# facebookresearch/seamless_communication

Measured on AMD Instinct MI355X. Metric: S2ST utterances/sec (and real-time factor), seamlessM4T_v2_large, 10 s audio, higher is better.
Workload: dtype f32 activations x f16 weights, f32 accumulate

## Files before the change

include/seamless_hip.h:

```cpp
#ifndef SEAMLESS_HIP_H_
#define SEAMLESS_HIP_H_

#include <stddef.h>
#include <stdint.h>

#ifdef __cplusplus
extern "C" {
#endif

#define SC_ABI_VERSION 10
#define SC_MAX_UPSAMPLES 8
#define SC_MAX_RESBLOCK_KERNELS 4
#define SC_MAX_RESBLOCK_DILATIONS 4

typedef enum sc_status {
    SC_OK = 0,
    SC_ERR_INVALID = -1,
    SC_ERR_HIP = -2,
    SC_ERR_CAPACITY = -3,
    SC_ERR_INTERNAL = -4
} sc_status;

typedef enum sc_dtype { SC_F16 = 0, SC_F32 = 1, SC_I32 = 2 } sc_dtype;

typedef struct sc_tensor_desc {
    const char* name;
    int32_t dtype;
    int32_t ndim;
    int64_t shape[4];
    const void* data;
    int32_t on_device;
} sc_tensor_desc;

typedef struct sc_config {
    int32_t abi_version;
    int32_t model_dim, num_heads;
    int32_t num_fbank_channels, fbank_stride;
    int32_t enc_layers, enc_ffn_dim, depthwise_conv_kernel_size, shaw_max_left, shaw_max_right;
    int32_t adaptor_kernel_size, adaptor_stride, adaptor_ffn_dim, adaptor_proj_dim;
    int32_t dec_layers, dec_ffn_dim, text_vocab_size, text_max_seq_len;
    int32_t pad_idx, unk_idx, bos_idx, eos_idx;
    int32_t t2u_enc_layers, t2u_dec_layers, t2u_ffn_dim, t2u_conv_kernel, t2u_conv_inner_dim;
    int32_t unit_vocab_size, unit_pad_idx, unit_eos_idx, unit_max_seq_len;
    int32_t char_vocab_size, char_max_seq_len, var_pred_hidden_dim, var_pred_kernel_size;
    int32_t voc_num_upsamples;
    int32_t voc_upsample_rates[SC_MAX_UPSAMPLES];
    int32_t voc_upsample_kernel_sizes[SC_MAX_UPSAMPLES];
    int32_t voc_upsample_initial_channel;
    int32_t voc_num_resblock_kernels;
    int32_t voc_resblock_kernel_sizes[SC_MAX_RESBLOCK_KERNELS];
    int32_t voc_num_resblock_dilations;
    int32_t voc_resblock_dilation_sizes[SC_MAX_RESBLOCK_KERNELS][SC_MAX_RESBLOCK_DILATIONS];
    int32_t voc_num_embeddings, voc_embedding_dim, voc_lang_embedding_dim, voc_num_langs;
    int32_t voc_spkr_embedding_dim, voc_num_spkrs;
    int32_t has_t2u, has_vocoder;
    int32_t text_enc_layers, text_enc_ffn_dim;
    int32_t mma_layers, mma_ffn_dim, mma_energy_layers, mma_pre_decision_ratio;
    float mma_temperature;
    int32_t enc_variant;
    int32_t voc_dur_pred_hidden_dim, voc_dur_pred_kernel_size;
    int32_t t2u_variant;
} sc_config;

typedef struct sc_gen_opts {
    int32_t beam_size;
    float soft_max_seq_len_a;
    int32_t soft_max_seq_len_b;
    int32_t hard_max_seq_len;
    int32_t min_seq_len;
    float unk_penalty;
    int32_t use_graph;
    float len_penalty;
    int32_t normalize_scores;
    int32_t no_repeat_ngram_size;
    int32_t source_len;
} sc_gen_opts;

typedef struct sc_model sc_model;

const char* sc_last_error(void);
int sc_abi_version(void);

sc_model* sc_load(const sc_tensor_desc* tensors, size_t n_tensors, const sc_config* cfg, int device);
sc_model* sc_fork(sc_model* parent);
void sc_free(sc_model* m);
int sc_synchronize(sc_model* m);
int sc_wait_stream(sc_model* m, void* producer_stream);
int sc_set_nar_tables(sc_model* m, int32_t vocab, const int32_t* h_tok_len, const uint8_t* h_starts_space,
                      const uint8_t* h_is_punct, const int64_t* h_char_offsets, const int32_t* h_char_ids);

int sc_fbank(sc_model* m, const float* d_wav, int32_t n, int64_t wav_stride, const int32_t* h_num_samples,
             int32_t standardize, float* d_out, int32_t t_rows, int32_t* h_out_frames);

// ... 112 lines not shown
```

include/seamless_hip_internal.h:

```cpp
#ifndef SEAMLESS_HIP_INTERNAL_H_
#define SEAMLESS_HIP_INTERNAL_H_

#include "seamless_hip.h"

#ifdef __cplusplus
extern "C" {
#endif

int sc_decoder_step_family(sc_model* m, int rows, int caller);

int sc_op_knob(const char* name, int dflt);

int sc_op_force_general_gemm(int on);
int32_t sc_op_voc_pack_plan(const int32_t* h_need, int32_t n, int64_t budget_rows, int32_t* h_group_first, int32_t cap);
int32_t sc_op_voc_tile_first(const int32_t* h_off, int32_t n, int32_t mul, int32_t tile_rows, int32_t* h_first);
int32_t sc_op_last_vocoder_packed_groups(sc_model* m);
int sc_op_single_plane(int on);
int sc_op_layernorm(const float* d_x, const float* d_gamma, const float* d_beta, float* d_y, int32_t rows, int32_t C,
                    int32_t act);
int sc_op_linear(const float* d_x, const void* d_w_f16, const float* d_bias, const float* d_res, float* d_y,
                 int32_t M, int32_t N, int32_t K, int32_t act, float alpha, int32_t split, int32_t force_gemv);
int sc_op_skinny_linear(const float* d_x, const void* d_w_f16, const float* d_bias, const float* d_res, float* d_y,
                        int32_t M, int32_t N, int32_t K, int32_t act, float alpha);
int sc_op_skinny_res_ln(const float* d_in, const void* d_w_f16, const float* d_bias, float* d_x_inout,
                        const float* d_gamma, const float* d_beta, float* d_h, int32_t M, int32_t N, int32_t K,
                        int32_t splits);
int sc_op_skinny_argmax(const float* d_x, const void* d_w_f16, int32_t M, int32_t N, int32_t K, int32_t step,
                        int32_t min_step_for_eos, int32_t force_eos_step, int32_t pad_idx, int32_t eos_idx,
                        int32_t unk_idx, float unk_penalty, int32_t* d_idx, float* d_lprob);

int sc_op_dstep_res_ln(const float* d_in, const void* d_w_f16, const float* d_bias, float* d_x_inout, const float* d_gamma,
                       const float* d_beta, float* d_h, int32_t M, int32_t N, int32_t K, int32_t splits);
int sc_op_dstep_linear_planes(const float* d_x, const void* d_w_f16, const float* d_bias, float* d_y, int32_t M, int32_t N, int32_t K,
                              int32_t act);
int sc_op_dstep_argmax(const float* d_x, const void* d_w_f16, int32_t M, int32_t N, int32_t K, int32_t step,
                       int32_t min_step_for_eos, int32_t force_eos_step, int32_t pad_idx, int32_t eos_idx, int32_t unk_idx,
                       float unk_penalty, int32_t ntl, int32_t* d_idx, float* d_lprob);
int sc_op_dstep_attention(const float* d_proj, int32_t S, const float* d_bias, float* d_kcache, float* d_vcache, int32_t cap,
                          int32_t pos, const int32_t* d_lens, int32_t cross, int32_t nb, int32_t heads, float* d_out);
int sc_op_dstep3_gemv(int32_t mode, const float* d_x, const void* d_w_f16, const float* d_bias, const float* d_gamma,
                      const float* d_beta, const float* d_res, float* d_y, float* d_h, int32_t M, int32_t N, int32_t K, int32_t act,
                      int32_t rg, int32_t shape);
int sc_op_dstep3_argmax(const float* d_x, const void* d_w_f16, int32_t M, int32_t N, int32_t K, int32_t step,
                        int32_t min_step_for_eos, int32_t force_eos_step, int32_t pad_idx, int32_t eos_idx, int32_t unk_idx,
                        float unk_penalty, int32_t* d_idx, float* d_lprob);
int sc_op_chain_bench(int32_t kind, int32_t rows, int32_t n, int32_t reps, float* us_per_kernel);
int sc_op_conv1d(const float* d_x, const void* d_w_f16_packed, const float* d_bias, const float* d_res, float* d_y,
                 int32_t nb, int32_t t_in, int32_t cin, int32_t cout, int32_t k, int32_t stride, int32_t pad,
                 int32_t dil, const int32_t* d_in_lens, int32_t in_act, int32_t act);
int sc_op_pack_conv_weight(const void* d_w_f16, void* d_dst_f16, int32_t cout, int32_t cin, int32_t k);
int sc_op_conv_transpose1d(const float* d_x, const void* d_v_f16, const void* d_g_f16, const float* d_bias,
                           float* d_y, int32_t nb, int32_t t_in, int32_t cin, int32_t cout, int32_t k,
                           int32_t stride, int32_t pad, int32_t in_act);
int sc_op_linear_presplit(const float* d_x, const void* d_w_f16, const float* d_bias, const float* d_res, float* d_y,
                          void* d_yh_f16, void* d_yl_f16, int32_t M, int32_t N, int32_t K, int32_t act, float alpha);
int sc_op_linear_presplit_argmax(const float* d_x, const void* d_w_f16, const float* d_bias, int32_t* d_idx, int32_t M, int32_t N,
                                 int32_t K);
int sc_op_conv1d_presplit(const float* d_x, const void* d_w_f16_packed, const float* d_bias, const float* d_res, float* d_y,
                          void* d_yh_f16, void* d_yl_f16, int32_t nb, int32_t t, int32_t cin, int32_t cout, int32_t k, int32_t pad,
                          int32_t dil, const unsigned char* d_row_valid, int32_t act);
int sc_op_resblock_pair_ps(const float* d_x, const void* d_w1_packed, const float* d_b1, const void* d_w2_packed, const float* d_b2,
                           float* d_out, int32_t nb, int32_t T, int32_t C, int32_t k, int32_t dil);
int sc_op_resblock_pair(const float* d_x, const void* d_w1_packed, const float* d_b1, const void* d_w2_packed,
                        const float* d_b2, float* d_out, int32_t nb, int32_t T, int32_t C, int32_t k, int32_t dil,
                        float slope, const float* d_avg_a, const float* d_avg_b);
int sc_op_mrf_fused(const float* d_x, const void* const* d_w1_packed, const float* const* d_b1, const void* const* d_w2_packed,
                    const float* const* d_b2, float* d_out, int32_t nb, int32_t T, int32_t C, const int32_t* k, const int32_t* dil,
                    float slope);
int sc_op_attention(const float* d_q, const float* d_k, const float* d_v, float* d_out, int32_t nb, int32_t heads,
                    int32_t sq, int32_t skv, int64_t ldq, int64_t ldk, int64_t ldv, int64_t ldo,
                    const int32_t* d_kv_lens, int32_t causal, const float* d_rel_k, int32_t rel_left,
                    int32_t rel_right);
int sc_op_attention_ex(const float* d_q, const float* d_k, const float* d_v, float* d_out, int32_t nb, int32_t heads,
                       int32_t sq, int32_t skv, int64_t ldq, int64_t ldk, int64_t ldv, int64_t ldo,
                       const int32_t* d_kv_lens, int32_t causal, const float* d_rel_k, int32_t rel_left,
                       int32_t rel_right, const int32_t* d_row_off, const float* d_rp_table, int64_t rp_ld,
                       const float* d_q_bias_u, const float* d_q_bias_v, void* d_out_hi, void* d_out_lo, int64_t ldoh);
int sc_op_glu_dwconv(const float* d_x, const float* d_w, float* d_y, int32_t nb, int32_t T, int32_t C, int32_t k,
                     const int32_t* d_lens);
int sc_op_glu_dwconv_ln(const float* d_x, const float* d_w, const float* d_gamma, const float* d_beta, int32_t act, void* d_yh_f16,
                        void* d_yl_f16, int32_t nb, int32_t T, int32_t C, int32_t k, const int32_t* d_lens, int32_t fused);
int sc_op_layernorm2(const float* d_x, const float* d_ga, const float* d_ba, const float* d_gb, const float* d_bb, float* d_y,
                     void* d_yh_f16, void* d_yl_f16, int32_t rows, int32_t C, int32_t fused);
int sc_op_argmax(const float* d_logits, int32_t rows, int32_t V, int32_t* d_idx, float* d_lprob);

int sc_op_beam_candidates(float* d_logits, int64_t ld, int32_t n_utt, int32_t beams, int32_t V, const float* d_cum, int32_t first_step,
                          int32_t no_eos, int32_t force_eos, int32_t pad_idx, int32_t eos_idx, int32_t unk_idx, float unk_penalty, int32_t K,
                          float* d_cand_val, int32_t* d_cand_idx, const int32_t* d_seqs, int32_t seq_ld, int32_t S, int32_t G,
                          const int32_t* d_rows, const int32_t* d_slots, int32_t chunked);
int sc_op_beam_candidates_banned(float* d_logits, int64_t ld, int32_t n_utt, int32_t beams, int32_t V, const float* d_cum,
                                 int32_t first_step, int32_t no_eos, int32_t force_eos, int32_t pad_idx, int32_t eos_idx, int32_t unk_idx,
                                 float unk_penalty, int32_t K, float* d_cand_val, int32_t* d_cand_idx, const int32_t* d_seqs,
                                 int32_t seq_ld, int32_t S, int32_t G, const int32_t* d_rows, const int32_t* d_slots, int32_t chunked,
                                 const int32_t* d_banned_tokens, const int32_t* d_banned_offsets, int32_t n_banned);
int sc_op_beam_select(const float* d_cand_val, const int32_t* d_cand_idx, const int32_t* d_seqs_cur, int32_t* d_seqs_new, float* d_fin_score,
                      int32_t* d_fin_len, int32_t* d_fin_seq, int32_t* d_fin_count, int32_t* d_done, int32_t* d_remaining, int32_t* d_tok,
                      int32_t* d_src_row, float* d_cum, int32_t* d_anc, int32_t anc_ld, const int32_t* d_slot_utt, const int32_t* d_slots,
                      int32_t n, int32_t beams, int32_t K, int32_t V, int32_t max_len, int32_t step, int32_t eos_idx, int32_t pad_idx,
                      int32_t normalize, float len_penalty);
int sc_op_beam_compact(const int32_t* d_done, int32_t* d_slot_utt, int32_t* d_slots, int32_t* d_rows, int32_t* d_seqs, float* d_cum,
                       int32_t* d_tok, int32_t* d_enc_lens, int32_t* d_anc, int32_t n, int32_t beams, int32_t max_len, int32_t anc_ld,
                       int32_t seq_len, int32_t anc_len);
int sc_op_gather_cache(const float* d_src, float* d_dst, const int32_t* d_src_row, int32_t rows, int32_t len, int32_t cap, int32_t M,
                       int32_t layers, int64_t layer_stride);
int sc_op_row_token_lprob(const float* d_logits, int64_t ld, int32_t rows, int32_t V, int32_t row_stride, int32_t token, float* d_out);

int sc_op_dstep_attention_ex(const float* d_proj, int32_t S, const float* d_bias, float* d_kcache, float* d_vcache, int32_t cap,
                             int32_t cache_rows, int32_t pos, const int32_t* d_lens, int32_t cross, int32_t nb, int32_t heads,
                             const int32_t* d_slot_rp, const int32_t* d_slot_lane, const int32_t* d_anc, const int32_t* d_kv_item,
                             int32_t kv_row_div, const int32_t* d_rows, float* d_out);
int sc_op_engine_step_close(const float* d_x, const void* d_w_f16, int32_t M, int32_t N, int32_t K, int32_t min_step_for_eos, int32_t pad_idx,
                            int32_t eos_idx, int32_t unk_idx, float unk_penalty, int32_t* d_slot_rp, const int32_t* d_rows, int32_t n_states,
                            int32_t cap, int32_t* d_tok, int32_t* d_pos, int32_t* d_finished, int32_t* d_out_len, const int32_t* d_limit,
                            const int32_t* d_prefix_len, float* d_score, int32_t* d_hist);
int sc_op_engine_admit(const int32_t* d_recs, int32_t n, int32_t n_states, int32_t cap, int32_t pad_idx, int32_t* d_tok, int32_t* d_pos,
                       int32_t* d_finished, int32_t* d_out_len, int32_t* d_limit, int32_t* d_prefix_len, int32_t* d_enc_lens, float* d_score,
                       int32_t* d_hist);
int sc_op_engine_set_slots(const int32_t* d_rids, int32_t n_live, int32_t slots, int32_t n_states, int32_t* d_slot_rp, int32_t* d_slot_lane,
                           const int32_t* d_pos, int32_t* d_rows);
int sc_op_engine_retire(const int32_t* h_rid, const int32_t* h_dst_rows, float* const* h_dst, int32_t n, int32_t n_states, int32_t cap, int32_t M,
                        const int32_t* d_out_len, const float* d_score, const int32_t* d_hist, const float* d_hidden, int32_t* d_stage);
int sc_op_dstep3_embed_ex(const int32_t* d_tok, const void* d_embed_f16, float scale, const float* d_pos_table, int32_t pos,
                          const int32_t* d_slot_rp, const int32_t* d_rows, int32_t rows, int32_t C, int32_t n_states, int32_t n_pos, int32_t vocab,
                          float* d_x);
int sc_op_dstep3_reduce_capture_ex(const float* d_partial, int32_t S, const float* d_bias, float* d_x_inout, const float* d_gamma, const float* d_beta,
                                   float* d_h, float* d_hrow, int64_t hrow_bs, int32_t hrow_rows, int32_t pos, const int32_t* d_slot_rp,
                                   const int32_t* d_rows, int32_t rows, int32_t C, int32_t n_states);
int sc_op_step_update(int32_t* d_next_tok, int32_t* d_hist, int32_t hist_ld, int32_t* d_finished, int32_t* d_out_len, const float* d_lprob,
                      float* d_score, int32_t nb, int32_t pos, int32_t pad_idx, int32_t eos_idx, int32_t* d_n_unfinished);
int sc_op_row_swap(float* d_k, float* d_v, float* d_cross, int32_t layers, int32_t pairs, const int32_t* h_src, const int32_t* h_dst, int32_t n_rows,
                   int32_t M, int32_t cap, int32_t s_enc, int32_t filled, int32_t* d_tok, int32_t* d_finished, int32_t* d_out_len,
                   int32_t* d_enc_lens, float* d_lprob, float* d_score, int32_t* d_hist, float* d_hidden);
int sc_op_align_lprob(const float* d_text, const float* d_feat, int32_t n, int32_t s_text, int32_t s_feat, int32_t C,
                      const int32_t* h_text_lens, const int32_t* h_feat_lens, float temperature, float* d_lprob);
int sc_op_mas(const float* d_lprob, int32_t n, int32_t s_text, int32_t s_feat, const int32_t* h_text_lens, const int32_t* h_feat_lens,
              int32_t* h_durations);

#ifdef __cplusplus
}
#endif
#endif
```

seamless_communication_amd/_lib.py:

```python
from __future__ import annotations

import ctypes as C
from pathlib import Path
from typing import Optional

import os

_VARIANT = os.environ.get("SC_LIB_VARIANT", "")
LIB_PATH = Path(__file__).resolve().parent / (f"libseamless_hip.{_VARIANT}.so" if _VARIANT else "libseamless_hip.so")

SC_ABI_VERSION = 10
SC_MAX_UPSAMPLES = 8
SC_MAX_RESBLOCK_KERNELS = 4
SC_MAX_RESBLOCK_DILATIONS = 4
SC_F16, SC_F32, SC_I32 = 0, 1, 2


class SeamlessHipError(RuntimeError):
    pass


class sc_tensor_desc(C.Structure):
    _fields_ = [
        ("name", C.c_char_p),
        ("dtype", C.c_int32),
        ("ndim", C.c_int32),
        ("shape", C.c_int64 * 4),
        ("data", C.c_void_p),
        ("on_device", C.c_int32),
    ]


_i = C.c_int32


class sc_config(C.Structure):
    _fields_ = [
        ("abi_version", _i), ("model_dim", _i), ("num_heads", _i),
        ("num_fbank_channels", _i), ("fbank_stride", _i),
        ("enc_layers", _i), ("enc_ffn_dim", _i), ("depthwise_conv_kernel_size", _i),
        ("shaw_max_left", _i), ("shaw_max_right", _i),
        ("adaptor_kernel_size", _i), ("adaptor_stride", _i), ("adaptor_ffn_dim", _i), ("adaptor_proj_dim", _i),
        ("dec_layers", _i), ("dec_ffn_dim", _i), ("text_vocab_size", _i), ("text_max_seq_len", _i),
        ("pad_idx", _i), ("unk_idx", _i), ("bos_idx", _i), ("eos_idx", _i),
        ("t2u_enc_layers", _i), ("t2u_dec_layers", _i), ("t2u_ffn_dim", _i), ("t2u_conv_kernel", _i),
        ("t2u_conv_inner_dim", _i),
        ("unit_vocab_size", _i), ("unit_pad_idx", _i), ("unit_eos_idx", _i), ("unit_max_seq_len", _i),
        ("char_vocab_size", _i), ("char_max_seq_len", _i), ("var_pred_hidden_dim", _i), ("var_pred_kernel_size", _i),
        ("voc_num_upsamples", _i),
        ("voc_upsample_rates", _i * SC_MAX_UPSAMPLES),
        ("voc_upsample_kernel_sizes", _i * SC_MAX_UPSAMPLES),
        ("voc_upsample_initial_channel", _i),
        ("voc_num_resblock_kernels", _i),
        ("voc_resblock_kernel_sizes", _i * SC_MAX_RESBLOCK_KERNELS),
        ("voc_num_resblock_dilations", _i),
        ("voc_resblock_dilation_sizes", (_i * SC_MAX_RESBLOCK_DILATIONS) * SC_MAX_RESBLOCK_KERNELS),
        ("voc_num_embeddings", _i), ("voc_embedding_dim", _i), ("voc_lang_embedding_dim", _i), ("voc_num_langs", _i),
        ("voc_spkr_embedding_dim", _i), ("voc_num_spkrs", _i),
        ("has_t2u", _i), ("has_vocoder", _i),
        ("text_enc_layers", _i), ("text_enc_ffn_dim", _i),
        ("mma_layers", _i), ("mma_ffn_dim", _i), ("mma_energy_layers", _i), ("mma_pre_decision_ratio", _i),
        ("mma_temperature", C.c_float),
        ("enc_variant", _i),
        ("voc_dur_pred_hidden_dim", _i), ("voc_dur_pred_kernel_size", _i),
        ("t2u_variant", _i),
    ]


class sc_gen_opts(C.Structure):
    _fields_ = [
        ("beam_size", _i), ("soft_max_seq_len_a", C.c_float), ("soft_max_seq_len_b", _i),
        ("hard_max_seq_len", _i), ("min_seq_len", _i), ("unk_penalty", C.c_float), ("use_graph", _i),
        ("len_penalty", C.c_float), ("normalize_scores", _i), ("no_repeat_ngram_size", _i), ("source_len", _i),
    ]


class sc_engine_opts(C.Structure):
    _fields_ = [
        ("slots", _i), ("rows", _i), ("max_len", _i), ("s_enc", _i), ("min_seq_len", _i), ("unk_penalty", C.c_float),
        ("poll", _i), ("low_water", _i), ("max_wait_ms", _i), ("use_graph", _i),
    ]


class sc_engine_stats(C.Structure):
    _fields_ = [
        ("steps", C.c_int64), ("row_steps", C.c_int64), ("useful_row_steps", C.c_int64), ("rows_admitted", C.c_int64),
        ("rows_retired", C.c_int64), ("requests", C.c_int64), ("max_live", C.c_int64), ("busy_us", C.c_double), ("wait_us", C.c_double),
        ("self_kv_bytes", C.c_int64), ("cross_kv_bytes", C.c_int64), ("hidden_bytes", C.c_int64),
    ]


class sc_aligner_config(C.Structure):
    _fields_ = [
        ("abi_version", _i), ("model_dim", _i), ("feat_dim", _i), ("text_layers", _i), ("feat_layers", _i),
# ... 8 lines not shown
    "sc_last_error": (C.c_char_p, []),
    "sc_abi_version": (C.c_int, []),
    "sc_load": (_P, [C.POINTER(sc_tensor_desc), C.c_size_t, C.POINTER(sc_config), C.c_int]),
    "sc_fork": (_P, [_P]),
    "sc_free": (None, [_P]),
    "sc_synchronize": (C.c_int, [_P]),
    "sc_wait_stream": (C.c_int, [_P, _P]),
    "sc_decoder_step_family": (C.c_int, [_P, C.c_int, C.c_int]),
    "sc_set_nar_tables": (C.c_int, [_P, _i, _P, _P, _P, _P, _P]),
    "sc_fbank": (C.c_int, [_P, _P, _i, C.c_int64, _P, _i, _P, _i, _P]),
    "sc_fbank_rate": (C.c_int, [_P, _P, _i, C.c_int64, _P, _i, _i, _P, _i, _P]),
    "sc_fbank_frames": (_i, [C.c_int64, _i]),
    "sc_encoder_out_len": (_i, [_P, _i]),
    "sc_encode_speech": (C.c_int, [_P, _P, _i, _i, _P, _P, _P]),
    "sc_encode_text": (C.c_int, [_P, _P, C.c_int32, C.c_int32, _P, _P]),
    "sc_mma_begin": (C.c_int, [_P, _P, C.c_int32, C.c_int32]),
    "sc_mma_step": (C.c_int, [_P, _P, C.c_int32, _P, C.c_int32, _P, _P, _P]),
    "sc_text_max_len": (_i, [_P, C.POINTER(sc_gen_opts), _i]),
    "sc_generate_text": (C.c_int, [_P, _P, _i, _i, _P, C.POINTER(sc_gen_opts), _P, _i, _P, _P, _P, _P]),
    "sc_generate_text_banned": (C.c_int, [_P, _P, _i, _i, _P, C.POINTER(sc_gen_opts), _P, _i, _P, _P, _P, _P, _P, _P, _i]),
    "sc_generate_text_capture": (C.c_int, [_P, _P, _i, _i, _P, C.POINTER(sc_gen_opts), _P, _i, _P, _P, _P, _P, _P, _P]),
    "sc_decode_text": (C.c_int, [_P, _P, _i, _i, _P, _P, _i, _P]),
    "sc_engine_create": (_P, [_P, C.POINTER(sc_engine_opts)]),
    "sc_engine_free": (None, [_P]),
    "sc_engine_attach": (C.c_int, [_P, _P]),
    "sc_engine_expect": (C.c_int, [_P, _i]),
    "sc_engine_get_stats": (C.c_int, [_P, C.POINTER(sc_engine_stats), _i]),
    "sc_t2u_nar": (C.c_int, [_P, _P, _i, _i, _P, _P, C.c_float, _P, _PI, _PI]),
    "sc_get_units": (C.c_int, [_P, _P]),
    "sc_get_durations": (C.c_int, [_P, _P, _P, _P]),
    "sc_vocoder_hop": (_i, [_P]),
    "sc_vocode": (C.c_int, [_P, _P, _i, _i, _P, _P, _P]),
    "sc_vocode_ragged": (C.c_int, [_P, _P, _i, _i, _P, _P, _P, _P]),
    "sc_vocoder_durations": (C.c_int, [_P, _P, _i, _i, _P]),
    "sc_t2u_ar": (C.c_int, [_P, _P, _i, _i, _P, C.POINTER(sc_gen_opts), _P, _i, _P, _i, _P, _P]),
    "sc_t2u_ar_max_len": (_i, [_P, C.POINTER(sc_gen_opts), _i]),
    "sc_last_padding": (C.c_int, [_P, _P, _P, _P]),
    "sc_s2st": (C.c_int, [_P, _P, _i, _i, _P, C.POINTER(sc_gen_opts), _P, _i, C.c_float, _P, _P, _P, _i, _P, _P, _i, _P, _P, _P]),
    "sc_prof_enable": (C.c_int, [C.c_int]),
    "sc_prof_reset": (C.c_int, []),
    "sc_prof_report": (C.c_int64, [C.c_char_p, C.c_int64]),
    "sc_text_to_char_seqs": (C.c_int32, [C.c_int32, _P, _P, _P, _P, _P, C.c_int32, C.c_int32, C.c_int32, _P, C.c_int32, C.c_int32,
                                         _P, _P, C.c_int32, _P]),
    "sc_ngram_blocked_tokens": (C.c_int32, [_PI, C.c_int32, C.c_int32, _PI, C.c_int32]),
    "sc_banned_blocked_tokens": (C.c_int32, [_PI, C.c_int32, _PI, _PI, C.c_int32, _PI, C.c_int32]),
    "sc_aligner_load": (_P, [C.POINTER(sc_tensor_desc), C.c_size_t, C.POINTER(sc_aligner_config), C.c_int]),
    "sc_aligner_free": (None, [_P]),
    "sc_align": (C.c_int, [_P, _P, _i, _i, _P, _P, _i, _P, _P, _P]),
    "sc_op_align_lprob": (C.c_int, [_P, _P, _i, _i, _i, _i, _P, _P, C.c_float, _P]),
    "sc_op_mas": (C.c_int, [_P, _i, _i, _i, _P, _P, _P]),
    "sc_op_knob": (C.c_int, [C.c_char_p, C.c_int]),
    "sc_op_force_general_gemm": (C.c_int, [C.c_int]),
    "sc_op_voc_pack_plan": (C.c_int32, [_PI, C.c_int32, C.c_int64, _PI, C.c_int32]),
    "sc_op_voc_tile_first": (C.c_int32, [_PI, C.c_int32, C.c_int32, C.c_int32, _PI]),
    "sc_op_last_vocoder_packed_groups": (C.c_int32, [_P]),
    "sc_op_single_plane": (C.c_int, [C.c_int]),
    "sc_op_layernorm": (C.c_int, [_P, _P, _P, _P, _i, _i, _i]),
    "sc_op_linear": (C.c_int, [_P, _P, _P, _P, _P, _i, _i, _i, _i, C.c_float, _i, _i]),
    "sc_op_skinny_linear": (C.c_int, [_P, _P, _P, _P, _P, _i, _i, _i, _i, C.c_float]),
    "sc_op_skinny_res_ln": (C.c_int, [_P, _P, _P, _P, _P, _P, _P, _i, _i, _i, _i]),
    "sc_op_skinny_argmax": (C.c_int, [_P, _P, _i, _i, _i, _i, _i, _i, _i, _i, _i, C.c_float, _P, _P]),
    "sc_op_dstep_res_ln": (C.c_int, [_P, _P, _P, _P, _P, _P, _P, _i, _i, _i, _i]),
    "sc_op_dstep_linear_planes": (C.c_int, [_P, _P, _P, _P, _i, _i, _i, _i]),
    "sc_op_dstep_argmax": (C.c_int, [_P, _P, _i, _i, _i, _i, _i, _i, _i, _i, _i, C.c_float, _i, _P, _P]),
    "sc_op_resblock_pair_ps": (C.c_int, [_P, _P, _P, _P, _P, _P, _i, _i, _i, _i, _i]),
    "sc_op_glu_dwconv_ln": (C.c_int, [_P, _P, _P, _P, _i, _P, _P, _i, _i, _i, _i, _P, _i]),
    "sc_op_layernorm2": (C.c_int, [_P, _P, _P, _P, _P, _P, _P, _P, _i, _i, _i]),
    "sc_op_dstep3_gemv": (C.c_int, [_i, _P, _P, _P, _P, _P, _P, _P, _P, _i, _i, _i, _i, _i, _i]),
    "sc_op_dstep3_argmax": (C.c_int, [_P, _P, _i, _i, _i, _i, _i, _i, _i, _i, _i, C.c_float, _P, _P]),
    "sc_op_chain_bench": (C.c_int, [_i, _i, _i, _i, _P]),
    "sc_op_dstep_attention": (C.c_int, [_P, _i, _P, _P, _P, _i, _i, _P, _i, _i, _i, _P]),
    "sc_op_conv1d": (C.c_int, [_P, _P, _P, _P, _P, _i, _i, _i, _i, _i, _i, _i, _i, _P, _i, _i]),
    "sc_op_pack_conv_weight": (C.c_int, [_P, _P, _i, _i, _i]),
    "sc_op_conv_transpose1d": (C.c_int, [_P, _P, _P, _P, _P, _i, _i, _i, _i, _i, _i, _i, _i]),
    "sc_op_linear_presplit": (C.c_int, [_P, _P, _P, _P, _P, _P, _P, _i, _i, _i, _i, C.c_float]),
    "sc_op_linear_presplit_argmax": (C.c_int, [_P, _P, _P, _P, _i, _i, _i]),
    "sc_op_conv1d_presplit": (C.c_int, [_P, _P, _P, _P, _P, _P, _P, _i, _i, _i, _i, _i, _i, _i, _P, _i]),
    "sc_op_mrf_fused": (C.c_int, [_P, _P, _P, _P, _P, _P, _i, _i, _i, _P, _P, C.c_float]),
    "sc_op_resblock_pair": (C.c_int, [_P, _P, _P, _P, _P, _P, _i, _i, _i, _i, _i, C.c_float, _P, _P]),
    "sc_op_attention": (C.c_int, [_P, _P, _P, _P, _i, _i, _i, _i, C.c_int64, C.c_int64, C.c_int64, C.c_int64, _P, _i,
                                  _P, _i, _i]),
    "sc_op_attention_ex": (C.c_int, [_P, _P, _P, _P, _i, _i, _i, _i, C.c_int64, C.c_int64, C.c_int64, C.c_int64, _P, _i,
                                     _P, _i, _i, _P, _P, C.c_int64, _P, _P, _P, _P, C.c_int64]),
    "sc_op_glu_dwconv": (C.c_int, [_P, _P, _P, _i, _i, _i, _i, _P]),
    "sc_op_argmax": (C.c_int, [_P, _i, _i, _P, _P]),
    "sc_op_beam_candidates": (C.c_int, [_P, C.c_int64, _i, _i, _i, _P, _i, _i, _i, _i, _i, _i, C.c_float, _i, _P, _P, _P, _i, _i, _i,
                                        _P, _P, _i]),
    "sc_op_beam_candidates_banned": (C.c_int, [_P, C.c_int64, _i, _i, _i, _P, _i, _i, _i, _i, _i, _i, C.c_float, _i, _P, _P, _P, _i, _i,
                                               _i, _P, _P, _i, _P, _P, _i]),
    "sc_op_beam_select": (C.c_int, [_P, _P, _P, _P, _P, _P, _P, _P, _P, _P, _P, _P, _P, _P, _i, _P, _P, _i, _i, _i, _i, _i, _i, _i, _i,
                                    _i, C.c_float]),
    "sc_op_beam_compact": (C.c_int, [_P, _P, _P, _P, _P, _P, _P, _P, _P, _i, _i, _i, _i, _i, _i]),
    "sc_op_gather_cache": (C.c_int, [_P, _P, _P, _i, _i, _i, _i, _i, C.c_int64]),
    "sc_op_row_token_lprob": (C.c_int, [_P, C.c_int64, _i, _i, _i, _i, _P]),
    "sc_op_dstep_attention_ex": (C.c_int, [_P, _i, _P, _P, _P, _i, _i, _i, _P, _i, _i, _i, _P, _P, _P, _P, _i, _P, _P]),
    "sc_op_engine_step_close": (C.c_int, [_P, _P, _i, _i, _i, _i, _i, _i, _i, C.c_float, _P, _P, _i, _i, _P, _P, _P, _P, _P, _P, _P, _P]),
    "sc_op_engine_admit": (C.c_int, [_P, _i, _i, _i, _i, _P, _P, _P, _P, _P, _P, _P, _P, _P]),
    "sc_op_engine_set_slots": (C.c_int, [_P, _i, _i, _i, _P, _P, _P, _P]),
    "sc_op_engine_retire": (C.c_int, [_P, _P, _P, _i, _i, _i, _i, _P, _P, _P, _P, _P]),
    "sc_op_dstep3_embed_ex": (C.c_int, [_P, _P, C.c_float, _P, _i, _P, _P, _i, _i, _i, _i, _i, _P]),
    "sc_op_dstep3_reduce_capture_ex": (C.c_int, [_P, _i, _P, _P, _P, _P, _P, _P, C.c_int64, _i, _i, _P, _P, _i, _i, _i]),
    "sc_op_step_update": (C.c_int, [_P, _P, _i, _P, _P, _P, _P, _i, _i, _i, _i, _P]),
    "sc_op_row_swap": (C.c_int, [_P, _P, _P, _i, _i, _P, _P, _i, _i, _i, _i, _i, _P, _P, _P, _P, _P, _P, _P, _P]),
}

_lib: Optional[C.CDLL] = None


def load_library() -> C.CDLL:
    global _lib
    if _lib is not None:
        return _lib
    if not LIB_PATH.exists():
        raise SeamlessHipError(
            f"{LIB_PATH} is missing: build it with `python -m seamless_communication_amd.build` "
            "(there is no CPU fallback for the HIP path)"
        )
    lib = C.CDLL(str(LIB_PATH))
    for name, (res, args) in SIGNATURES.items():
        fn = getattr(lib, name)
        fn.restype = res
        fn.argtypes = args
    if lib.sc_abi_version() != SC_ABI_VERSION:
        raise SeamlessHipError(f"ABI mismatch: library {lib.sc_abi_version()} vs binding {SC_ABI_VERSION}")
    _lib = lib
    return lib


def banned_csr(banned_seqs):
    import numpy as np

    seqs = [[int(t) for t in (s.tolist() if hasattr(s, "tolist") else s)] for s in banned_seqs]
    if any(len(s) == 0 for s in seqs):
        raise ValueError("a banned sequence must hold at least one token")
    off = np.zeros(len(seqs) + 1, dtype=np.int32)
    off[1:] = np.cumsum([len(s) for s in seqs], dtype=np.int64)
    tok = np.asarray([t for s in seqs for t in s], dtype=np.int32)
    return tok, off


def check(status: int, what: str) -> None:
    if status != 0:
        msg = load_library().sc_last_error()
        raise SeamlessHipError(f"{what} failed with status {status}: {msg.decode() if msg else '?'}")


def make_config(cfg, has_t2u: bool = True, has_vocoder: bool = True, has_text_encoder: bool = False,
                has_monotonic_decoder: bool = False, has_vocoder_dur_predictor: bool = False) -> sc_config:
    c = sc_config()
    c.abi_version = SC_ABI_VERSION
    for f in (
        "model_dim num_heads num_fbank_channels fbank_stride enc_layers enc_ffn_dim depthwise_conv_kernel_size "
        "shaw_max_left shaw_max_right adaptor_kernel_size adaptor_stride adaptor_ffn_dim adaptor_proj_dim dec_layers "
        "dec_ffn_dim text_vocab_size text_max_seq_len pad_idx unk_idx bos_idx eos_idx t2u_enc_layers t2u_dec_layers "
        "t2u_ffn_dim t2u_conv_kernel t2u_conv_inner_dim unit_vocab_size unit_pad_idx unit_eos_idx unit_max_seq_len "
        "char_vocab_size char_max_seq_len var_pred_hidden_dim var_pred_kernel_size"
    ).split():
        setattr(c, f, int(getattr(cfg, f)))
    v = cfg.vocoder
    if len(v.upsample_rates) > SC_MAX_UPSAMPLES or len(v.resblock_kernel_sizes) > SC_MAX_RESBLOCK_KERNELS:
        raise ValueError("vocoder config exceeds the ABI's fixed array sizes")
    c.voc_num_upsamples = len(v.upsample_rates)
    for i, (r, k) in enumerate(zip(v.upsample_rates, v.upsample_kernel_sizes)):
        c.voc_upsample_rates[i] = r
        c.voc_upsample_kernel_sizes[i] = k
    c.voc_upsample_initial_channel = v.upsample_initial_channel
# ... 30 lines not shown
```

seamless_communication_amd/csrc/api.hip:

```cpp
#include <atomic>
#include <cstring>
#include <map>
#include <mutex>
#include <set>

#include "../../include/seamless_hip_internal.h"
#include "engine.h"
#include "model.h"

using namespace sc;

struct sc_model {
    Model m;
};

struct sc_engine {
    std::unique_ptr<Engine> e;
    int device = 0;
    const void* weights = nullptr;
    std::set<sc_model*> attached;
};

static std::mutex g_attach_mu;
static std::map<Engine*, sc_engine*> g_engine_owner;
// ... 1030 lines not shown
        if (kind == 7) one(i & 1 ? 1 : 2);
        else one(kind);
    }
    SC_HIP(hipStreamEndCapture(st, &g));
    SC_HIP(hipGraphInstantiate(&ge, g, nullptr, nullptr, 0));
    for (int r = 0; r < 2; ++r) SC_HIP(hipGraphLaunch(ge, st));
    SC_HIP(hipStreamSynchronize(st));
    hipEvent_t e0, e1;
    SC_HIP(hipEventCreate(&e0));
    SC_HIP(hipEventCreate(&e1));
    SC_HIP(hipEventRecord(e0, st));
    for (int r = 0; r < reps; ++r) SC_HIP(hipGraphLaunch(ge, st));
    SC_HIP(hipEventRecord(e1, st));
    SC_HIP(hipStreamSynchronize(st));
    float ms = 0.f;
    SC_HIP(hipEventElapsedTime(&ms, e0, e1));
    *us_per_kernel = 1e3f * ms / (float)(reps * n);
    (void)hipEventDestroy(e0);
    (void)hipEventDestroy(e1);
    (void)hipGraphExecDestroy(ge);
    (void)hipGraphDestroy(g);
    (void)hipStreamDestroy(st);
    SC_API_END
}

int sc_op_pack_conv_weight(const void* d_w_f16, void* d_dst_f16, int32_t cout, int32_t cin, int32_t k) {
    SC_API_BEGIN
    const int kpad = (int)align_up((int64_t)cin * k, 32);
    launch_pack_conv_weight(static_cast<const __half*>(d_w_f16), static_cast<__half*>(d_dst_f16), cout, cin, k, kpad,
                            g_op_stream);
    SC_HIP(hipStreamSynchronize(g_op_stream));
    SC_API_END
}

int sc_op_conv1d(const float* d_x, const void* d_w_f16_packed, const float* d_bias, const float* d_res, float* d_y,
                 int32_t nb, int32_t t_in, int32_t cin, int32_t cout, int32_t k, int32_t stride, int32_t pad, int32_t dil,
                 const int32_t* d_in_lens, int32_t in_act, int32_t act) {
    SC_API_BEGIN
    Model tmp;
    Conv c;
    c.w = static_cast<const __half*>(d_w_f16_packed);
    c.b = d_bias;
    c.cout = cout;
    c.cin = cin;
    c.k = k;
    c.kpad = (int)align_up((int64_t)cin * k, 32);
    conv1d(tmp, d_x, c, d_res, d_y, nb, t_in, stride, pad, dil, d_in_lens, in_act, act);
    SC_HIP(hipStreamSynchronize(g_op_stream));
    SC_API_END
}

int sc_op_conv_transpose1d(const float* d_x, const void* d_v_f16, const void* d_g_f16, const float* d_bias, float* d_y,
                           int32_t nb, int32_t t_in, int32_t cin, int32_t cout, int32_t k, int32_t stride, int32_t pad,
                           int32_t in_act) {
    SC_API_BEGIN
    SC_CHECK(pad == (k - stride) / 2 && k - 2 * pad == stride, "sc_op_conv_transpose1d: unsupported geometry");
    Model tmp;
    ConvT c;
    c.cin = cin;
    c.cout = cout;
    c.k = k;
    c.stride = stride;
    c.pad = pad;
    c.taps = cdiv(k, stride);
    c.kpad = (int)align_up((int64_t)cin * c.taps, 32);
    float* folded = nullptr;
    __half* packed = nullptr;
    SC_HIP(hipMalloc(&folded, (size_t)cin * cout * k * 4));
    SC_HIP(hipMalloc(&packed, (size_t)stride * cout * c.kpad * 2));
    launch_weight_norm_fold(static_cast<const __half*>(d_v_f16), static_cast<const __half*>(d_g_f16), folded, cin, cout * k,
                            g_op_stream);
    launch_pack_convT_weight(folded, packed, cin, cout, k, stride, c.kpad, g_op_stream);
    c.w = packed;
    c.b = d_bias;
    conv_transpose1d(tmp, d_x, c, d_y, nb, t_in, in_act);
    SC_HIP(hipStreamSynchronize(g_op_stream));
    (void)hipFree(folded);
    (void)hipFree(packed);
    SC_API_END
}

int sc_op_linear_presplit(const float* d_x, const void* d_w_f16, const float* d_bias, const float* d_res, float* d_y,
                          void* d_yh_f16, void* d_yl_f16, int32_t M, int32_t N, int32_t K, int32_t act, float alpha) {
    SC_API_BEGIN
    SC_CHECK(d_x && d_w_f16 && (d_y || d_yh_f16), "sc_op_linear_presplit: null argument");
    __half *hi = nullptr, *lo = nullptr;
    SC_HIP(hipMalloc(&hi, (size_t)M * K * 2));
    SC_HIP(hipMalloc(&lo, (size_t)M * K * 2));
    try {
        launch_split_f32(d_x, hi, lo, (int64_t)M * K, g_op_stream);
        GemmPsArgs a;
        a.Ah = hi;
        a.Al = lo;
        a.lda = K;
        a.W = static_cast<const __half*>(d_w_f16);
        a.ldw = K;
        a.bias = d_bias;
        a.res = d_res;
        a.ldr = N;
        a.C = d_y;
        a.ldc = N;
        a.Ch = static_cast<__half*>(d_yh_f16);
        a.Cl = static_cast<__half*>(d_yl_f16);
        a.ldcs = N;
        a.M = M;
        a.N = N;
        a.K = K;
        a.act = act;
        a.alpha = alpha;
        launch_gemm_presplit(a, g_op_stream);
        SC_HIP(hipStreamSynchronize(g_op_stream));
    } catch (...) {
        (void)hipFree(hi);
        (void)hipFree(lo);
        throw;
    }
    (void)hipFree(hi);
    (void)hipFree(lo);
    SC_API_END
}

int sc_op_linear_presplit_argmax(const float* d_x, const void* d_w_f16, const float* d_bias, int32_t* d_idx, int32_t M, int32_t N,
                                 int32_t K) {
    SC_API_BEGIN
    SC_CHECK(d_x && d_w_f16 && d_idx, "sc_op_linear_presplit_argmax: null argument");
    __half *hi = nullptr, *lo = nullptr;
    float2* part = nullptr;
    const int nch = gemm_presplit_amax_chunks(M, N);
    SC_HIP(hipMalloc(&hi, (size_t)M * K * 2));
    SC_HIP(hipMalloc(&lo, (size_t)M * K * 2));
    SC_HIP(hipMalloc(&part, (size_t)M * nch * sizeof(float2)));
    try {
        SC_HIP(hipMemsetAsync(part, 0xff, (size_t)M * nch * sizeof(float2), g_op_stream));
        launch_split_f32(d_x, hi, lo, (int64_t)M * K, g_op_stream);
        GemmPsArgs a;
        a.Ah = hi;
        a.Al = lo;
        a.lda = K;
        a.W = static_cast<const __half*>(d_w_f16);
        a.ldw = K;
        a.bias = d_bias;
        a.M = M;
        a.N = N;
        a.K = K;
        a.amax = part;
        a.amax_ld = nch;
        launch_gemm_presplit(a, g_op_stream);
        launch_amax_finish(part, nch, M, d_idx, g_op_stream);
        SC_HIP(hipStreamSynchronize(g_op_stream));
    } catch (...) {
        (void)hipFree(hi);
        (void)hipFree(lo);
        (void)hipFree(part);
        throw;
    }
    (void)hipFree(hi);
    (void)hipFree(lo);
    (void)hipFree(part);
    SC_API_END
}

int sc_op_conv1d_presplit(const float* d_x, const void* d_w_f16_packed, const float* d_bias, const float* d_res, float* d_y,
                          void* d_yh_f16, void* d_yl_f16, int32_t nb, int32_t t, int32_t cin, int32_t cout, int32_t k, int32_t pad,
                          int32_t dil, const unsigned char* d_row_valid, int32_t act) {
    SC_API_BEGIN
    SC_CHECK(d_x && d_w_f16_packed && (d_y || d_yh_f16), "sc_op_conv1d_presplit: null argument");
    __half *hi = nullptr, *lo = nullptr;
    const size_t n = (size_t)nb * t * cin;
    SC_HIP(hipMalloc(&hi, n * 2));
    SC_HIP(hipMalloc(&lo, n * 2));
    try {
        launch_split_f32(d_x, hi, lo, (int64_t)n, g_op_stream);
        Model tmp;
        Conv c;
        c.w = static_cast<const __half*>(d_w_f16_packed);
        c.b = d_bias;
        c.cout = cout;
        c.cin = cin;
        c.k = k;
        c.kpad = (int)align_up((int64_t)cin * k, 32);
        conv1d_presplit(tmp, hi, lo, c, d_res, d_y, static_cast<__half*>(d_yh_f16), static_cast<__half*>(d_yl_f16), nb, t, pad, dil,
                        d_row_valid, act);
        SC_HIP(hipStreamSynchronize(g_op_stream));
    } catch (...) {
        (void)hipFree(hi);
        (void)hipFree(lo);
        throw;
// ... 55 lines not shown
int sc_op_mrf_fused(const float* d_x, const void* const* d_w1_packed, const float* const* d_b1, const void* const* d_w2_packed,
                    const float* const* d_b2, float* d_out, int32_t nb, int32_t T, int32_t C, const int32_t* k, const int32_t* dil,
                    float slope) {
    SC_API_BEGIN
    SC_CHECK(d_x && d_w1_packed && d_b1 && d_w2_packed && d_b2 && d_out && k && dil, "sc_op_mrf_fused: null argument");
    MrfArgs a;
    a.x = d_x;
    a.out = d_out;
    a.nb = nb;
    a.T = T;
    a.C = C;
    a.slope = slope;
    for (int j = 0; j < 3; ++j) a.k[j] = k[j];
    for (int q = 0; q < 9; ++q) {
        a.dil[q] = dil[q];
        a.w1[q] = static_cast<const __half*>(d_w1_packed[q]);
        a.w2[q] = static_cast<const __half*>(d_w2_packed[q]);
        a.ldw1[q] = a.ldw2[q] = align_up((int64_t)C * k[q / 3], 32);
        a.b1[q] = d_b1[q];
        a.b2[q] = d_b2[q];
    }
    a.single = g_op_single.load();
    launch_mrf_fused(a, g_op_stream);
    SC_HIP(hipStreamSynchronize(g_op_stream));
    SC_API_END
}

int sc_op_attention(const float* d_q, const float* d_k, const float* d_v, float* d_out, int32_t nb, int32_t heads,
                    int32_t sq, int32_t skv, int64_t ldq, int64_t ldk, int64_t ldv, int64_t ldo, const int32_t* d_kv_lens,
                    int32_t causal, const float* d_rel_k, int32_t rel_left, int32_t rel_right) {
    SC_API_BEGIN
    AttnArgs a;
    a.q = d_q;
    a.k = d_k;
    a.v = d_v;
    a.out = d_out;
    a.ldq = ldq;
    a.ldk = ldk;
    a.ldv = ldv;
    a.ldo = ldo;
    a.nb = nb;
    a.heads = heads;
    a.Sq = sq;
    a.Skv = skv;
    a.kv_lens = d_kv_lens;
    a.causal = causal;
    a.rel_k = d_rel_k;
    a.rel_left = rel_left;
    a.rel_right = rel_right;
    launch_attention(a, g_op_stream);
    SC_HIP(hipStreamSynchronize(g_op_stream));
    SC_API_END
}

int sc_op_attention_ex(const float* d_q, const float* d_k, const float* d_v, float* d_out, int32_t nb, int32_t heads,
                       int32_t sq, int32_t skv, int64_t ldq, int64_t ldk, int64_t ldv, int64_t ldo, const int32_t* d_kv_lens,
                       int32_t causal, const float* d_rel_k, int32_t rel_left, int32_t rel_right, const int32_t* d_row_off,
                       const float* d_rp_table, int64_t rp_ld, const float* d_q_bias_u, const float* d_q_bias_v, void* d_out_hi,
                       void* d_out_lo, int64_t ldoh) {
    SC_API_BEGIN
    AttnArgs a;
    a.q = d_q;
    a.k = d_k;
    a.v = d_v;
    a.out = d_out;
    a.ldq = ldq;
    a.ldk = ldk;
    a.ldv = ldv;
    a.ldo = ldo;
    a.nb = nb;
    a.heads = heads;
    a.Sq = sq;
    a.Skv = skv;
    a.kv_lens = d_kv_lens;
    a.causal = causal;
    a.rel_k = d_rel_k;
    a.rel_left = rel_left;
    a.rel_right = rel_right;
    a.row_off = d_row_off;
    a.rp_table = d_rp_table;
    a.rp_ld = rp_ld;
    a.q_bias_u = d_q_bias_u;
    a.q_bias_v = d_q_bias_v;
    a.out_hi = static_cast<__half*>(d_out_hi);
    a.out_lo = static_cast<__half*>(d_out_lo);
    a.ldoh = ldoh;
    launch_attention(a, g_op_stream);
    SC_HIP(hipStreamSynchronize(g_op_stream));
    SC_API_END
}

int sc_op_glu_dwconv(const float* d_x, const float* d_w, float* d_y, int32_t nb, int32_t T, int32_t C, int32_t k,
                     const int32_t* d_lens) {
    SC_API_BEGIN
    launch_glu_dwconv(d_x, 2 * C, d_w, d_y, C, nb, T, C, k, d_lens, g_op_stream);
    SC_HIP(hipStreamSynchronize(g_op_stream));
    SC_API_END
}

int sc_op_glu_dwconv_ln(const float* d_x, const float* d_w, const float* d_gamma, const float* d_beta, int32_t act, void* d_yh_f16,
                        void* d_yl_f16, int32_t nb, int32_t T, int32_t C, int32_t k, const int32_t* d_lens, int32_t fused) {
    SC_API_BEGIN
    SC_CHECK(d_x && d_w && d_gamma && d_beta && d_yh_f16 && d_yl_f16, "sc_op_glu_dwconv_ln: null argument");
    __half* yh = static_cast<__half*>(d_yh_f16);
    __half* yl = static_cast<__half*>(d_yl_f16);
    if (fused) {
        launch_glu_dwconv_ln(d_x, 2 * C, d_w, d_gamma, d_beta, act, yh, yl, C, nb, T, C, k, d_lens, g_op_stream);
    } else {
        OpScratch scratch;
        float* mid = scratch.get<float>((size_t)nb * T * C);
        launch_glu_dwconv(d_x, 2 * C, d_w, mid, C, nb, T, C, k, d_lens, g_op_stream);
        launch_layernorm_split(mid, C, d_gamma, d_beta, yh, yl, C, nb * T, C, act, nullptr, 1, g_op_stream);
        SC_HIP(hipStreamSynchronize(g_op_stream));
    }
    SC_HIP(hipStreamSynchronize(g_op_stream));
    SC_API_END
}

int sc_op_layernorm2(const float* d_x, const float* d_ga, const float* d_ba, const float* d_gb, const float* d_bb, float* d_y,
                     void* d_yh_f16, void* d_yl_f16, int32_t rows, int32_t C, int32_t fused) {
    SC_API_BEGIN
    SC_CHECK(d_x && d_ga && d_ba && d_gb && d_bb && d_y && d_yh_f16 && d_yl_f16, "sc_op_layernorm2: null argument");
    __half* yh = static_cast<__half*>(d_yh_f16);
    __half* yl = static_cast<__half*>(d_yl_f16);
    if (fused) {
        launch_layernorm2_split(d_x, C, d_ga, d_ba, d_y, C, d_gb, d_bb, yh, yl, C, rows, C, g_op_stream);
    } else {
        launch_layernorm(d_x, C, d_ga, d_ba, d_y, C, rows, C, ACT_NONE, nullptr, 1, g_op_stream);
        launch_layernorm_split(d_y, C, d_gb, d_bb, yh, yl, C, rows, C, ACT_NONE, nullptr, 1, g_op_stream);
    }
    SC_HIP(hipStreamSynchronize(g_op_stream));
    SC_API_END
}

int sc_op_argmax(const float* d_logits, int32_t rows, int32_t V, int32_t* d_idx, float* d_lprob) {
    SC_API_BEGIN
    launch_argmax_rows(d_logits, V, rows, V, nullptr, -1, -1, -1, -1, -1, 0.f, d_idx, d_lprob, g_op_stream);
    SC_HIP(hipStreamSynchronize(g_op_stream));
    SC_API_END
}


static int op_beam_candidates(float* d_logits, int64_t ld, int32_t n_utt, int32_t beams, int32_t V, const float* d_cum, int32_t first_step,
                              int32_t no_eos, int32_t force_eos, int32_t pad_idx, int32_t eos_idx, int32_t unk_idx, float unk_penalty, int32_t K,
                              float* d_cand_val, int32_t* d_cand_idx, const int32_t* d_seqs, int32_t seq_ld, int32_t S, int32_t G,
                              const int32_t* d_rows, const int32_t* d_slots, int32_t chunked, const int32_t* d_banned_tokens,
                              const int32_t* d_banned_offsets, int32_t n_banned) {
    SC_API_BEGIN
    BannedList bl;
    if (n_banned != 0) {
        SC_CHECK(n_banned > 0 && n_banned <= BANNED_MAX_SEQS && d_banned_tokens && d_banned_offsets && d_seqs,
                 "sc_op_beam_candidates_banned: bad banned list (n_banned=%d; needs d_seqs)", n_banned);
        const std::vector<int32_t> off = op_read_ints(d_banned_offsets, (size_t)n_banned + 1);
        SC_CHECK(off[0] == 0 && off[n_banned] >= 0 && off[n_banned] <= BANNED_MAX_TOKENS, "sc_op_beam_candidates_banned: bad offsets");
        for (int q = 0; q < n_banned; ++q) SC_CHECK(off[q + 1] >= off[q], "sc_op_beam_candidates_banned: offsets decrease at %d", q);
        const std::vector<int32_t> tok = op_read_ints(d_banned_tokens, (size_t)off[n_banned]);
        validate_banned_host(tok.data(), off.data(), n_banned, V, &bl.max_len);
        bl.tokens = d_banned_tokens, bl.offsets = d_banned_offsets, bl.n = n_banned;
    }
    const BannedList* banned = bl.n > 0 ? &bl : nullptr;
    SC_CHECK(d_logits && d_cum && d_cand_val && d_cand_idx && n_utt >= 1 && V >= 1 && ld >= V, "sc_op_beam_candidates: bad arguments");
    SC_CHECK(!d_seqs || (G >= 0 && S >= 0 && seq_ld >= S), "sc_op_beam_candidates: bad n-gram arguments (S=%d G=%d seq_ld=%d)", S, G, seq_ld);
    if (d_slots) SC_CHECK(op_read_ints(d_slots, 1)[0] <= n_utt, "sc_op_beam_candidates: *d_slots > n_utt");
    if (chunked) {
        SC_CHECK(beam_chunked(V, beams, K), "sc_op_beam_candidates: the chunked search does not take V=%d beams=%d K=%d", V, beams, K);
        if (d_rows) SC_CHECK(op_read_ints(d_rows, 1)[0] <= n_utt * beams, "sc_op_beam_candidates: *d_rows > n_utt * beams");
// ... 384 lines not shown
```

seamless_communication_amd/csrc/common.cpp:

```cpp
#include "common.h"
#include <cstdlib>
#include <cstring>

namespace sc {

static thread_local char g_err[1024] = "";

void set_error(const char* fmt, ...) {
    va_list ap;
    va_start(ap, fmt);
    vsnprintf(g_err, sizeof(g_err), fmt, ap);
    va_end(ap);
}

const char* get_error() { return g_err; }

namespace knob {
namespace {
struct Knob {
    const char* name;
    int kind;
    const char* what;
};
const Knob knob_table[] = {
    {"SC_DEBUG_NUMERICS", 0, "honour the switches that change results"},
    {"SC_DEBUG_FILL", 0, "fill fresh scratch blocks with NaN (tests)"},
    {"SC_SPLIT_MODE", 1, "1: Conformer products on the hi fp16 plane only (precision study)"},
    {"SC_DECODER_GEN1", 1, "decoder step on the first-generation kernels"},
    {"SC_DECODER_GEN2", 1, "decoder step on the second-generation chain"},
    {"SC_DECODE_STEPWISE", 1, "teacher-forced pass step by step instead of one batched forward"},
    {"SC_VOC_SPLIT", 1, "vocoder ResBlock products on both fp16 planes of their activations again (bit 0 wide stages, bit 2 narrow stages); default: hi plane only"},
    {"SC_GEMM_GENERAL", 0, "general GEMM kernel instead of the fast path"}, {"SC_GEMM_PF2", 0, "GEMM prefetch depth"},
    {"SC_GEMM_GROUP_M", 0, "GEMM workgroup order"}, {"SC_GEMM_TILE", 0, "GEMM tile override"},
    {"SC_PS_TILE", 0, "DMA GEMM: largest tile"}, {"SC_PS_MIN256", 0, "DMA GEMM: tiles needed for 256 x 256"},
    {"SC_PS_MIN128", 0, "DMA GEMM: tiles needed for 128 x 128"},
    {"SC_PRESPLIT", 0, "0: Conformer operands split on the fly"}, {"SC_ENC_FUSE", 0, "0: separate Conformer element-wise launches"},
    {"SC_D3_RG_SMALL", 0, "decoder step: rows per row group, N = 1024 products"}, {"SC_D3_RG_FFN", 0, "decoder step: rows per row group, FFN-in"},
    {"SC_G3_STATIONARY", 0, "row-group products of wide steps: 0 one workgroup per row group, n = workgroup budget of the weight-stationary launch"},
    {"SC_G3_TILES", 0, "0: FFN-out of wide steps on the weight-stationary row-group walk instead of tile-owning waves"},
    {"SC_G3_TOUCH", 0, "weight-stationary products: bit 0 cooperative L2 touch of the activations, bit 1 K slices per XCD (FFN-out); default 3"},
    {"SC_D3_FFN_IN", 0, "decoder step: FFN-in workgroup shape"}, {"SC_D3_FFN_OUT", 0, "decoder step: FFN-out workgroup shape"},
    {"SC_T2U_GROUPS", 0, "NAR T2U: length buckets"}, {"SC_T2U_PACKED", 0, "0: NAR decoder on padded buckets"},
    {"SC_VOC_PS", 0, "0: vocoder wide stages on the register-staged convolution"}, {"SC_VOC_MRF", 0, "0: narrow vocoder stages as nine pair launches"},
    {"SC_VOC_GROUPS", 0, "vocoder: length buckets"}, {"SC_VOC_GROUP_OVERHEAD", 0, "vocoder: bucket planning overhead rows"},
    {"SC_VOC_STREAMS", 0, "vocoder: side chains"},
    {"SC_VOC_PACKED", 0, "0: ragged vocoder batches in length buckets on side chains instead of the packed pass"},
    {"SC_VOC_PACK_ROWS", 0, "vocoder: unit rows per packed group"},
    {"SC_ENGINE_RG_SMALL", 0, "decode engine: rows per row group, N = 1024 products"},
    {"SC_BEAM_COMPACT", 2, "0: beam search keeps finished utterances' slots"},
    {"SC_GREEDY_COMPACT", 2, "0: greedy generation keeps finished rows in their slots"}, {"SC_GREEDY_POLL", 2, "steps between looks at the finished flags"},
};
constexpr int N_KNOBS = sizeof(knob_table) / sizeof(knob_table[0]);
struct State {
    bool set[N_KNOBS];
    int val[N_KNOBS];
    bool numerics = false;
};
const State& state() {
    static const State st = [] {
        State s{};
        const char* dn = getenv("SC_DEBUG_NUMERICS");
        s.numerics = dn && atoi(dn) != 0;
        for (int i = 0; i < N_KNOBS; ++i) {
            const char* e = getenv(knob_table[i].name);
            s.set[i] = e != nullptr && (knob_table[i].kind != 1 || s.numerics);
            s.val[i] = e ? atoi(e) : 0;
        }
        return s;
    }();
    return st;
}
int lookup(const char* name) {
    for (int i = 0; i < N_KNOBS; ++i)
        if (strcmp(knob_table[i].name, name) == 0) return i;
    return -1;
}
int find(const char* name) {
    const int i = lookup(name);
    if (i >= 0) return i;
    fprintf(stderr, "libseamless_hip: switch %s is not in the knob table (common.cpp)\n", name);
    abort();
}
}

bool known(const char* name) { return name && lookup(name) >= 0; }

int value(const char* name, int dflt) {
    const int i = find(name);
    return state().set[i] ? state().val[i] : dflt;
}
bool is_set(const char* name) { return state().set[find(name)]; }
int live(const char* name, int dflt) {
    (void)find(name);
    const char* e = getenv(name);
    return e ? atoi(e) : dflt;
}
void report_once() {
    static const bool done = [] {
        const State& s = state();
        for (int i = 0; i < N_KNOBS; ++i) {
            const char* e = getenv(knob_table[i].name);
            if (!e || knob_table[i].kind == 2) continue;
            if (knob_table[i].kind == 1 && !s.numerics)
                fprintf(stderr, "libseamless_hip: %s=%s IGNORED - it changes results (%s); set SC_DEBUG_NUMERICS=1 to honour it\n", knob_table[i].name, e,
                        knob_table[i].what);
            else
                fprintf(stderr, "libseamless_hip: %s=%s (%s)%s\n", knob_table[i].name, e, knob_table[i].what, knob_table[i].kind == 1 ? " - RESULTS CHANGE" : "");
        }
        return true;
    }();
    (void)done;
}
}

}
```

seamless_communication_amd/csrc/k_attn.hip:

```cpp
#include <cstdlib>

#include "kernels.h"

namespace sc {

static constexpr int HD = 64;

static constexpr int MQ = 128;
static constexpr int MKV = 32;
static constexpr int KS = 68;
typedef _Float16 a16_h8 __attribute__((ext_vector_type(8)));
typedef _Float16 a16_h4 __attribute__((ext_vector_type(4)));
static constexpr int KH_LD = 72;
static constexpr int VT_LD = 40;

__device__ __forceinline__ void a16_split8(const float* x, a16_h8& hi, a16_h8& lo) {
#pragma unroll
    for (int e = 0; e < 8; ++e) {
        const _Float16 h = (_Float16)x[e];
        hi[e] = h;
        lo[e] = (_Float16)(x[e] - (float)h);
    }
}

template <int MODE>
__global__ __launch_bounds__(256) void attn_mfma16_kernel(AttnArgs p) {
    constexpr bool SHAW = MODE == 1;
    constexpr bool RELPOS = MODE == 2;
    typedef float f16v __attribute__((ext_vector_type(16)));
    typedef float f4v __attribute__((ext_vector_type(4)));
    extern __shared__ __attribute__((aligned(16))) float smem[];
    _Float16* sKh = reinterpret_cast<_Float16*>(smem);
    _Float16* sKl = sKh + MKV * KH_LD;
    _Float16* sVh = sKl + MKV * KH_LD;
    _Float16* sVl = sVh + HD * VT_LD;
    float* sQR = smem + 4 * 32 * KS;
    float* sT = smem + 4 * 32 * KS;
    float* sR = smem;

    const int tid = threadIdx.x, lane = tid & 63, wave = tid >> 6;
    const int ql = lane & 31, hh = lane >> 5;
    int qb = blockIdx.x, h = blockIdx.y, n = blockIdx.z;
    {
        const int gx = gridDim.x, bh_all = gridDim.y * gridDim.z;
        if ((bh_all & 7) == 0) {
            const int L = blockIdx.x + gx * (blockIdx.y + gridDim.y * blockIdx.z);
            const int bh = (L / (8 * gx)) * 8 + (L & 7);
            qb = (L >> 3) % gx;
            h = bh % gridDim.y;
            n = bh / gridDim.y;
        }
    }
    const int q0 = qb * MQ + wave * 32;
    const int qi = q0 + ql;
    const int kv_len = p.kv_lens ? min(p.kv_lens[n], p.Skv) : p.Skv;
    const int shift = p.Skv - p.Sq;
    const int qabs = qi + shift;
    const int npos = p.rel_left + 1 + p.rel_right;
    const int sq_n = p.row_off ? kv_len : p.Sq;
    const int64_t qbase = p.row_off ? (int64_t)p.row_off[n] : (int64_t)n * p.Sq;
    const int64_t kvbase = p.row_off ? (int64_t)p.row_off[n] : (int64_t)n * p.Skv;
    if (p.row_off && qb * MQ >= kv_len) return;
    const bool qok = qi < sq_n;
    const float* qrow = p.q + (qbase + (qok ? qi : 0)) * p.ldq + h * HD;

    if (SHAW) {
        float qreg[32];
#pragma unroll
        for (int g = 0; g < 8; ++g) {
            f4v v = {0.f, 0.f, 0.f, 0.f};
            if (qok) v = *reinterpret_cast<const f4v*>(qrow + 8 * g + 4 * hh);
            qreg[4 * g + 0] = v[0];
            qreg[4 * g + 1] = v[1];
            qreg[4 * g + 2] = v[2];
            qreg[4 * g + 3] = v[3];
        }
        for (int idx = tid; idx < npos * (HD / 4); idx += 256) {
            const int r = idx >> 4, c4 = idx & 15;
            *reinterpret_cast<f4v*>(&sR[r * KS + c4 * 4]) = *reinterpret_cast<const f4v*>(p.rel_k + r * HD + c4 * 4);
        }
        __syncthreads();
#pragma unroll 1
        for (int f = 0; f < 3; ++f) {
            if (f * 32 >= npos) break;
            f16v qr;
#pragma unroll
            for (int r = 0; r < 16; ++r) qr[r] = 0.f;
#pragma unroll
            for (int g = 0; g < 8; ++g) {
                const f4v r4 = *reinterpret_cast<const f4v*>(&sR[(f * 32 + ql) * KS + 8 * g + 4 * hh]);
                qr = __builtin_amdgcn_mfma_f32_32x32x2f32(r4[0], qreg[4 * g + 0], qr, 0, 0, 0);
                qr = __builtin_amdgcn_mfma_f32_32x32x2f32(r4[1], qreg[4 * g + 1], qr, 0, 0, 0);
                qr = __builtin_amdgcn_mfma_f32_32x32x2f32(r4[2], qreg[4 * g + 2], qr, 0, 0, 0);
                qr = __builtin_amdgcn_mfma_f32_32x32x2f32(r4[3], qreg[4 * g + 3], qr, 0, 0, 0);
            }
#pragma unroll
            for (int r = 0; r < 16; ++r) {
                const int e = f * 32 + (r & 3) + 8 * (r >> 2) + 4 * hh;
                if (e < npos) sQR[(wave * 32 + ql) * npos + e] = qr[r];
            }
        }
    }

    a16_h8 qh[4], qlo[4], qvh[RELPOS ? 4 : 1], qvl[RELPOS ? 4 : 1];
#pragma unroll
    for (int c = 0; c < 4; ++c) {
        float x[8];
#pragma unroll
        for (int e = 0; e < 8; ++e) x[e] = 0.f;
        if (qok) {
            const f4v v0 = *reinterpret_cast<const f4v*>(qrow + 16 * c + 8 * hh);
            const f4v v1 = *reinterpret_cast<const f4v*>(qrow + 16 * c + 8 * hh + 4);
#pragma unroll
            for (int e = 0; e < 4; ++e) {
                x[e] = v0[e];
                x[4 + e] = v1[e];
            }
        }
        if (RELPOS) {
            float xu[8], xv[8];
#pragma unroll
            for (int e = 0; e < 8; ++e) {
                xu[e] = x[e] + p.q_bias_u[h * HD + 16 * c + 8 * hh + e];
                xv[e] = x[e] + p.q_bias_v[h * HD + 16 * c + 8 * hh + e];
            }
            a16_split8(xu, qh[c], qlo[c]);
            a16_split8(xv, qvh[c], qvl[c]);
        } else {
            a16_split8(x, qh[c], qlo[c]);
        }
    }

    f16v o0, o1;
#pragma unroll
    for (int r = 0; r < 16; ++r) {
        o0[r] = 0.f;
        o1[r] = 0.f;
    }
    float m_i = -1e30f, l_i = 0.f;

    int k_end = kv_len;
    if (p.causal) k_end = min(k_end, qb * MQ + MQ - 1 + shift + 1);

    const int sr0 = tid >> 4, sc4 = tid & 15;
    f4v kf[2], vf[2];
    auto fetch = [&](int k0) {
#pragma unroll
        for (int u = 0; u < 2; ++u) {
            const int r = sr0 + 16 * u;
            kf[u] = f4v{0.f, 0.f, 0.f, 0.f};
            vf[u] = kf[u];
            if (k0 + r < kv_len) {
                const int64_t row = kvbase + k0 + r;
                kf[u] = *reinterpret_cast<const f4v*>(p.k + row * p.ldk + h * HD + sc4 * 4);
                vf[u] = *reinterpret_cast<const f4v*>(p.v + row * p.ldv + h * HD + sc4 * 4);
            }
        }
    };
    if (k_end > 0) fetch(0);

    for (int k0 = 0; k0 < k_end; k0 += MKV) {
        __syncthreads();
#pragma unroll
        for (int u = 0; u < 2; ++u) {
            const int r = sr0 + 16 * u;
            a16_h4 khi, klo, vhi, vlo;
#pragma unroll
            for (int e = 0; e < 4; ++e) {
                const _Float16 a = (_Float16)kf[u][e];
                khi[e] = a;
                klo[e] = (_Float16)(kf[u][e] - (float)a);
                const _Float16 b = (_Float16)vf[u][e];
                vhi[e] = b;
                vlo[e] = (_Float16)(vf[u][e] - (float)b);
            }
            *reinterpret_cast<a16_h4*>(&sKh[r * KH_LD + 4 * sc4]) = khi;
            *reinterpret_cast<a16_h4*>(&sKl[r * KH_LD + 4 * sc4]) = klo;
            const int w = r & 15;
            const int pos = (r & 16) + 8 * ((w >> 2) & 1) + (w & 3) + 4 * (w >> 3);
#pragma unroll
            for (int e = 0; e < 4; ++e) {
                sVh[(4 * sc4 + e) * VT_LD + pos] = vhi[e];
                sVl[(4 * sc4 + e) * VT_LD + pos] = vlo[e];
            }
        }
        if (k0 + MKV < k_end) fetch(k0 + MKV);
        __syncthreads();

        float qr[16];
        if (SHAW) {
            const float* qrow_t = sQR + (wave * 32 + ql) * npos;
            const int rel_max = k0 + (MKV - 1) - (q0 + shift);
            const int rel_min = k0 - (q0 + 31 + shift);
            if (rel_max <= -p.rel_left) {
                const float v = qrow_t[0];
#pragma unroll
                for (int r = 0; r < 16; ++r) qr[r] = v;
            } else if (rel_min >= p.rel_right) {
                const float v = qrow_t[npos - 1];
#pragma unroll
                for (int r = 0; r < 16; ++r) qr[r] = v;
            } else {
#pragma unroll
                for (int r = 0; r < 16; ++r) {
                    const int kj = k0 + (r & 3) + 8 * (r >> 2) + 4 * hh;
                    const int rel = max(-p.rel_left, min(p.rel_right, kj - qabs)) + p.rel_left;
                    qr[r] = qrow_t[rel];
                }
            }
        }
        if (RELPOS) {
            const int t0w = (p.Skv - 1) - (q0 + shift) + k0 - 31;
            const int t_max = 2 * p.Skv - 2;
            float* tw = sT + wave * (64 * 32);
#pragma unroll
            for (int blk = 0; blk < 2; ++blk) {
                const int trow = min(max(t0w + blk * 32 + ql, 0), t_max);
                const float* rrow = p.rp_table + (int64_t)trow * p.rp_ld + h * HD + 8 * hh;
                f4v ra[4][2];
#pragma unroll
                for (int c = 0; c < 4; ++c) {
                    ra[c][0] = *reinterpret_cast<const f4v*>(rrow + 16 * c);
                    ra[c][1] = *reinterpret_cast<const f4v*>(rrow + 16 * c + 4);
                }
                f16v tt;
#pragma unroll
                for (int r = 0; r < 16; ++r) tt[r] = 0.f;
#pragma unroll
                for (int c = 0; c < 4; ++c) {
                    float x[8];
#pragma unroll
                    for (int e = 0; e < 4; ++e) {
                        x[e] = ra[c][0][e];
                        x[4 + e] = ra[c][1][e];
                    }
                    a16_h8 rh, rl;
                    a16_split8(x, rh, rl);
                    tt = __builtin_amdgcn_mfma_f32_32x32x16_f16(rh, qvh[c], tt, 0, 0, 0);
                    tt = __builtin_amdgcn_mfma_f32_32x32x16_f16(rh, qvl[c], tt, 0, 0, 0);
                    tt = __builtin_amdgcn_mfma_f32_32x32x16_f16(rl, qvh[c], tt, 0, 0, 0);
                }
#pragma unroll
                for (int r = 0; r < 16; ++r) tw[(blk * 32 + (r & 3) + 8 * (r >> 2) + 4 * hh) * 32 + ql] = tt[r];
            }
#pragma unroll
            for (int r = 0; r < 16; ++r) {
                const int jl = (r & 3) + 8 * (r >> 2) + 4 * hh;
                qr[r] = tw[(jl - ql + 31) * 32 + ql];
            }
        }
        f16v st;
#pragma unroll
        for (int r = 0; r < 16; ++r) st[r] = 0.f;
#pragma unroll
        for (int c = 0; c < 4; ++c) {
            const a16_h8 kh = *reinterpret_cast<const a16_h8*>(&sKh[ql * KH_LD + 16 * c + 8 * hh]);
            const a16_h8 kl = *reinterpret_cast<const a16_h8*>(&sKl[ql * KH_LD + 16 * c + 8 * hh]);
            st = __builtin_amdgcn_mfma_f32_32x32x16_f16(kh, qh[c], st, 0, 0, 0);
            st = __builtin_amdgcn_mfma_f32_32x32x16_f16(kh, qlo[c], st, 0, 0, 0);
            st = __builtin_amdgcn_mfma_f32_32x32x16_f16(kl, qh[c], st, 0, 0, 0);
        }
        float mx = -INFINITY;
#pragma unroll
        for (int r = 0; r < 16; ++r) {
            const int kj = k0 + (r & 3) + 8 * (r >> 2) + 4 * hh;
            float sc = st[r];
            if (SHAW || RELPOS) sc += qr[r];
            const bool ok = (kj < kv_len) && (!p.causal || kj <= qabs);
            sc = sc * 0.125f + (ok ? 0.f : -INFINITY);
            st[r] = sc;
            mx = fmaxf(mx, sc);
        }
        mx = fmaxf(mx, __shfl_xor(mx, 32));
        const float m_new = fmaxf(m_i, mx);
        constexpr float LOG2E = 1.44269504088896340736f;
        const float alpha = __builtin_amdgcn_exp2f((m_i - m_new) * LOG2E);
        float rs = 0.f;
#pragma unroll
        for (int r = 0; r < 16; ++r) {
            const float pv = __builtin_amdgcn_exp2f((st[r] - m_new) * LOG2E);
            st[r] = pv;
            rs += pv;
        }
        rs += __shfl_xor(rs, 32);
        l_i = l_i * alpha + rs;
        m_i = m_new;
        if (__builtin_amdgcn_ballot_w64(alpha != 1.f) != 0) {
#pragma unroll
            for (int r = 0; r < 16; ++r) {
                o0[r] *= alpha;
                o1[r] *= alpha;
            }
        }
#pragma unroll
        for (int c = 0; c < 2; ++c) {
            float x[8];
#pragma unroll
            for (int e = 0; e < 8; ++e) x[e] = st[8 * c + e];
            a16_h8 ph, pl;
            a16_split8(x, ph, pl);
            const a16_h8 v0h = *reinterpret_cast<const a16_h8*>(&sVh[ql * VT_LD + 16 * c + 8 * hh]);
            const a16_h8 v0l = *reinterpret_cast<const a16_h8*>(&sVl[ql * VT_LD + 16 * c + 8 * hh]);
            const a16_h8 v1h = *reinterpret_cast<const a16_h8*>(&sVh[(32 + ql) * VT_LD + 16 * c + 8 * hh]);
            const a16_h8 v1l = *reinterpret_cast<const a16_h8*>(&sVl[(32 + ql) * VT_LD + 16 * c + 8 * hh]);
            o0 = __builtin_amdgcn_mfma_f32_32x32x16_f16(v0h, ph, o0, 0, 0, 0);
            o1 = __builtin_amdgcn_mfma_f32_32x32x16_f16(v1h, ph, o1, 0, 0, 0);
            o0 = __builtin_amdgcn_mfma_f32_32x32x16_f16(v0h, pl, o0, 0, 0, 0);
            o1 = __builtin_amdgcn_mfma_f32_32x32x16_f16(v1h, pl, o1, 0, 0, 0);
            o0 = __builtin_amdgcn_mfma_f32_32x32x16_f16(v0l, ph, o0, 0, 0, 0);
            o1 = __builtin_amdgcn_mfma_f32_32x32x16_f16(v1l, ph, o1, 0, 0, 0);
        }
    }

    __syncthreads();
    float* ot = smem + wave * (32 * KS);
    const float inv = l_i > 0.f ? 1.0f / l_i : 0.f;
#pragma unroll
    for (int r = 0; r < 16; ++r) {
        const int d = (r & 3) + 8 * (r >> 2) + 4 * hh;
        ot[ql * KS + d] = o0[r] * inv;
        ot[ql * KS + 32 + d] = o1[r] * inv;
    }
#pragma unroll
    for (int it = 0; it < 8; ++it) {
        const int row = it * 4 + (lane >> 4);
        const int c0 = (lane & 15) * 4;
        const int qq = q0 + row;
        const f4v of = *reinterpret_cast<const f4v*>(&ot[row * KS + c0]);
        if (qq >= sq_n) continue;
        if (p.out_hi) {
            const a16_h4 hi = __builtin_convertvector(of, a16_h4);
            const f4v back = __builtin_convertvector(hi, f4v);
            const int64_t off = (qbase + qq) * p.ldoh + h * HD + c0;
            *reinterpret_cast<a16_h4*>(p.out_hi + off) = hi;
            *reinterpret_cast<a16_h4*>(p.out_lo + off) = __builtin_convertvector(of - back, a16_h4);
        } else {
            *reinterpret_cast<f4v*>(p.out + (qbase + qq) * p.ldo + h * HD + c0) = of;
        }
    }
}

static bool g_attn_attr_set = false;

void launch_attention(const AttnArgs& a, hipStream_t s) {
    SC_CHECK(a.nb > 0 && a.heads > 0 && a.Sq > 0 && a.Skv > 0, "attention: empty problem");
    SC_CHECK(a.out || (a.out_hi && a.out_lo && a.ldoh % 4 == 0), "attention: no output");
    SC_CHECK(a.ldq % 4 == 0 && a.ldk % 4 == 0 && a.ldv % 4 == 0 && a.ldo % 4 == 0 && (reinterpret_cast<uintptr_t>(a.out) & 15) == 0,
             "attention: row strides must be multiples of 4 and the output 16-byte aligned");
    const int npos = a.rel_left + 1 + a.rel_right;
    SC_CHECK(npos <= 96, "attention: %d relative positions > 96", npos);
    SC_CHECK(!a.row_off || (a.kv_lens && a.Sq == a.Skv && !a.causal), "attention: packed rows need kv_lens and Sq == Skv");
    if (a.rp_table)
        SC_CHECK(!a.rel_k && !a.causal && a.Sq == a.Skv && a.q_bias_u && a.q_bias_v && a.rp_ld % 4 == 0,
                 "attention: relative positions need self-attention (Sq == Skv), both query biases and a 16-byte aligned table");
    if (!g_attn_attr_set) {
        SC_HIP(hipFuncSetAttribute(reinterpret_cast<const void*>(&attn_mfma16_kernel<0>), hipFuncAttributeMaxDynamicSharedMemorySize, 120 * 1024));
        SC_HIP(hipFuncSetAttribute(reinterpret_cast<const void*>(&attn_mfma16_kernel<1>), hipFuncAttributeMaxDynamicSharedMemorySize, 120 * 1024));
        SC_HIP(hipFuncSetAttribute(reinterpret_cast<const void*>(&attn_mfma16_kernel<2>), hipFuncAttributeMaxDynamicSharedMemorySize, 120 * 1024));
        g_attn_attr_set = true;
    }
    const double pairs = a.pairs > 0 ? a.pairs : (double)a.nb * a.Sq * a.Skv;
    prof::Scope scope(a.rel_k ? "attention_shaw" : "attention", 4.0 * a.heads * pairs * HD,
                      4.0 * a.nb * a.heads * HD * (2.0 * a.Sq + 2.0 * a.Skv), s);
    size_t lds = (size_t)(4 * 32 * KS) * sizeof(float);
    if (a.rel_k) lds += (size_t)(MQ * npos) * sizeof(float);
    if (a.rp_table) lds += (size_t)(4 * 64 * 32) * sizeof(float);
    dim3 grid(cdiv(a.Sq, MQ), a.heads, a.nb);
    if (a.rp_table) hipLaunchKernelGGL((attn_mfma16_kernel<2>), grid, dim3(256), lds, s, a);
    else if (a.rel_k) hipLaunchKernelGGL((attn_mfma16_kernel<1>), grid, dim3(256), lds, s, a);
    else hipLaunchKernelGGL((attn_mfma16_kernel<0>), grid, dim3(256), lds, s, a);
    SC_LAUNCH_CHECK();
}

static constexpr int MAX_CACHE = 4096;

__global__ __launch_bounds__(256) void decode_attn_kernel(
    const float* __restrict__ q, int64_t ldq, const float* __restrict__ k_new,
    const float* __restrict__ v_new, int64_t ldkv, float* __restrict__ kcache,
    float* __restrict__ vcache, int64_t cache_ld, int64_t cache_bs, int cap, float* __restrict__ out,
    int64_t ldo, int heads, const int* __restrict__ d_pos, const int* __restrict__ kv_lens, int use_lens,
    int in_splits, int64_t in_split_stride, const float* __restrict__ bias_q,
    const float* __restrict__ bias_k, const float* __restrict__ bias_v) {
    __shared__ float s_q[HD];
    __shared__ float s_sc[MAX_CACHE];
    __shared__ float s_red[8];
    __shared__ float s_part[4][HD];

    const int tid = threadIdx.x, lane = tid & 63, wave = tid >> 6;
    const int h = blockIdx.x, b = blockIdx.y;
    const int pos = d_pos ? *d_pos : 0;
    const int kv_len = use_lens ? min(kv_lens[b], cap) : pos + 1;
    float* kc = kcache + (int64_t)b * cache_bs + h * HD;
    float* vc = vcache + (int64_t)b * cache_bs + h * HD;
    if (tid < 3 * HD) {
        const int which = tid >> 6, d = tid & 63;
        if (which == 0 || k_new) {
            const float* src = which == 0 ? q : (which == 1 ? k_new : v_new);
            const int64_t ld = which == 0 ? ldq : ldkv;
            const float* bias = which == 0 ? bias_q : (which == 1 ? bias_k : bias_v);
            float v = 0.f;
            for (int sp = 0; sp < in_splits; ++sp) v += src[(int64_t)sp * in_split_stride + (int64_t)b * ld + h * HD + d];
            if (bias) v += bias[h * HD + d];
            if (which == 0) s_q[d] = v;
            else if (which == 1) kc[(int64_t)pos * cache_ld + d] = v;
            else vc[(int64_t)pos * cache_ld + d] = v;
        }
    }
    __syncthreads();
    const int sub = lane & 15, grp = lane >> 4;
    const float4 q4 = *reinterpret_cast<const float4*>(&s_q[sub * 4]);
    float lmax = -INFINITY;
    for (int j0 = 0; j0 < kv_len; j0 += 16) {
        const int j = j0 + wave * 4 + grp;
        float d = 0.f;
        if (j < kv_len) {
            const float4 kv = *reinterpret_cast<const float4*>(kc + (int64_t)j * cache_ld + sub * 4);
            d = fmaf(q4.x, kv.x, d);
            d = fmaf(q4.y, kv.y, d);
            d = fmaf(q4.z, kv.z, d);
            d = fmaf(q4.w, kv.w, d);
        }
#pragma unroll
        for (int off = 8; off > 0; off >>= 1) d += __shfl_xor(d, off);
        if (j < kv_len) {
            d *= 0.125f;
            if (sub == 0) s_sc[j] = d;
            lmax = fmaxf(lmax, d);
        }
    }
#pragma unroll
    for (int off = 32; off > 0; off >>= 1) lmax = fmaxf(lmax, __shfl_xor(lmax, off));
    if (lane == 0) s_red[wave] = lmax;
    __syncthreads();
    const float mx = fmaxf(fmaxf(s_red[0], s_red[1]), fmaxf(s_red[2], s_red[3]));
    float lsum = 0.f;
    for (int j = tid; j < kv_len; j += 256) {
        const float e = expf(s_sc[j] - mx);
        s_sc[j] = e;
        lsum += e;
    }
#pragma unroll
    for (int off = 32; off > 0; off >>= 1) lsum += __shfl_xor(lsum, off);
    if (lane == 0) s_red[4 + wave] = lsum;
    __syncthreads();
    const float denom = (s_red[4] + s_red[5]) + (s_red[6] + s_red[7]);
    float acc = 0.f;
    for (int j = wave; j < kv_len; j += 4) acc = fmaf(s_sc[j], vc[(int64_t)j * cache_ld + lane], acc);
    s_part[wave][lane] = acc;
    __syncthreads();
    if (tid < HD) {
        const float v = (s_part[0][tid] + s_part[1][tid]) + (s_part[2][tid] + s_part[3][tid]);
// ... 20 lines not shown
```

seamless_communication_amd/csrc/k_gemm_ps.hip:

```cpp
#include <cstdlib>
#include <type_traits>

#include "kernels.h"

namespace sc {

typedef _Float16 half8_t __attribute__((ext_vector_type(8)));
typedef float float16_t __attribute__((ext_vector_type(16)));

namespace {

constexpr int PBK = 32;
#define SC_LDS_PTR(p) ((__attribute__((address_space(3))) void*)(p))

template <int ACT>
__device__ __forceinline__ float ps_act(float v) {
    if (ACT == ACT_RELU) return v > 0.f ? v : 0.f;
    if (ACT == ACT_SILU) return v / (1.f + expf(-v));
    if (ACT == ACT_TANH) return tanhf(v);
    return v;
}

typedef int i32x4_t __attribute__((ext_vector_type(4)));

__device__ __forceinline__ i32x4_t make_rsrc_words(const void* base, uint32_t bytes) {
    const uint64_t b = reinterpret_cast<uint64_t>(base);
    i32x4_t r;
    r[0] = __builtin_amdgcn_readfirstlane((int)(uint32_t)b);
    r[1] = __builtin_amdgcn_readfirstlane((int)(uint32_t)((b >> 32) & 0xffff));
    r[2] = __builtin_amdgcn_readfirstlane((int)bytes);
    r[3] = 0x00020000;
    return r;
}

__device__ __forceinline__ int swz(int row, int s) { return row * 64 + ((s ^ ((row >> 2) & 3)) << 4); }

template <int WM, int WN, int EP_LD, int ACT>
__device__ __forceinline__ void ps_epilogue(const GemmPsArgs& p, const float* ep, int m0w, int n0w, int lane) {
    typedef float f4_t __attribute__((ext_vector_type(4)));
    typedef _Float16 h4_t __attribute__((ext_vector_type(4)));
    constexpr int LPR = WN / 4;
    constexpr int RPG = 16 / LPR;
    constexpr int RPI = 4 * RPG;
    const int l5 = lane & 31;
    const bool g1 = (l5 >= 4 && l5 < 12) || (l5 >= 16 && l5 < 20) || l5 >= 28;
    const int rank = g1 ? (l5 < 12 ? l5 - 4 : l5 < 20 ? l5 - 8 : l5 - 16) : (l5 < 4 ? l5 : l5 < 16 ? l5 - 8 : l5 - 12);
    const int grp = (lane >> 5) * 2 + (g1 ? 1 : 0);
    const int row_in = grp * RPG + rank / LPR;
    const int c0 = (rank % LPR) * 4;
    const int col = n0w + c0;
    const bool vec_ok = (col + 3 < p.N) && ((p.ldc | p.ldr | p.ldcs) % 4 == 0) && (n0w % 4 == 0);
    f4_t b4 = {0.f, 0.f, 0.f, 0.f};
    if (p.bias) {
#pragma unroll
        for (int e = 0; e < 4; ++e) b4[e] = (col + e < p.N) ? p.bias[col + e] : 0.f;
    }
#pragma unroll
    for (int it = 0; it < WM / RPI; ++it) {
        const int row = it * RPI + row_in;
        const int64_t m = m0w + row;
        const f4_t a = *reinterpret_cast<const f4_t*>(ep + row * EP_LD + c0);
        if (m >= p.M || col >= p.N) continue;
        const bool dead = p.row_valid && p.row_valid[m] == 0;
        f4_t v;
#pragma unroll
        for (int e = 0; e < 4; ++e) v[e] = dead ? 0.f : ps_act<ACT>(a[e] + b4[e]) * p.alpha;
        if (vec_ok) {
            if (p.res && !dead) v += *reinterpret_cast<const f4_t*>(p.res + m * p.ldr + col);
            if (p.C) *reinterpret_cast<f4_t*>(p.C + m * p.ldc + col) = v;
            if (p.Ch) {
                if (p.plane_neg_slope != 1.0f) {
#pragma unroll
                    for (int e = 0; e < 4; ++e) v[e] = fmaxf(v[e], 0.f) + p.plane_neg_slope * fminf(v[e], 0.f);
                }
                const h4_t hi = __builtin_convertvector(v, h4_t);
                *reinterpret_cast<h4_t*>(reinterpret_cast<_Float16*>(p.Ch) + m * p.ldcs + col) = hi;
                if (p.Cl)
                    *reinterpret_cast<h4_t*>(reinterpret_cast<_Float16*>(p.Cl) + m * p.ldcs + col) =
                        __builtin_convertvector(v - __builtin_convertvector(hi, f4_t), h4_t);
            }
        } else {
#pragma unroll
            for (int e = 0; e < 4; ++e) {
                if (col + e >= p.N) continue;
                float x = v[e];
                if (p.res && !dead) x += p.res[m * p.ldr + col + e];
                if (p.C) p.C[m * p.ldc + col + e] = x;
                if (p.Ch) {
                    if (p.plane_neg_slope != 1.0f) x = fmaxf(x, 0.f) + p.plane_neg_slope * fminf(x, 0.f);
                    const _Float16 h = (_Float16)x;
                    reinterpret_cast<_Float16*>(p.Ch)[m * p.ldcs + col + e] = h;
                    if (p.Cl) reinterpret_cast<_Float16*>(p.Cl)[m * p.ldcs + col + e] = (_Float16)(x - (float)h);
                }
            }
        }
    }
}

template <int BM, int BN, int WGM, int WGN, bool SPLIT, bool CONV, bool AMAX>
__global__ __launch_bounds__(WGM* WGN * 64) void gemm_ps_kernel(GemmPsArgs p, int tiles_n, int tiles_total, int tiles_per_xcd,
                                                                 uint32_t a_bytes, uint32_t w_bytes) {
    constexpr int NWAVE = WGM * WGN;
    constexpr bool ALTERNATE = SPLIT && NWAVE == 8;
    constexpr bool MID_BARRIER = SPLIT && !ALTERNATE;
    constexpr int WM = BM / WGM, WN = BN / WGN;
    constexpr int TM = WM / 32, TN = WN / 32;
    constexpr int ACH = BM / (16 * NWAVE);
    constexpr int BCH = BN / (16 * NWAVE);
    constexpr uint32_t OOB = 0x80000000u;
    constexpr int A_TILE = BM * 32, B_TILE = BN * 32;

    constexpr int A_PL = SPLIT ? 2 : 1;
    constexpr int STAGE_BYTES = (A_PL * A_TILE + B_TILE) * 2;
    constexpr int EPN = WN < 64 ? WN : (NWAVE * WM * (64 + 4) * 4 <= 3 * STAGE_BYTES ? 64 : 32);
    constexpr int EP_LD = EPN + 4;
    static_assert(NWAVE * WM * EP_LD * 4 <= 3 * STAGE_BYTES, "epilogue tiles must fit in the stage memory");
    __shared__ __attribute__((aligned(16))) char smem[3 * STAGE_BYTES];
    _Float16* const sAh0 = reinterpret_cast<_Float16*>(smem);
    _Float16* const sAl0 = sAh0 + (A_PL - 1) * A_TILE;
    _Float16* const sB0 = sAh0 + A_PL * A_TILE;
    _Float16* const sAh1 = reinterpret_cast<_Float16*>(smem + STAGE_BYTES);
    _Float16* const sAl1 = sAh1 + (A_PL - 1) * A_TILE;
    _Float16* const sB1 = sAh1 + A_PL * A_TILE;
    _Float16* const sAh2 = reinterpret_cast<_Float16*>(smem + 2 * STAGE_BYTES);
    _Float16* const sAl2 = sAh2 + (A_PL - 1) * A_TILE;
    _Float16* const sB2 = sAh2 + A_PL * A_TILE;

    const int bid = blockIdx.x;
    const int tile = (bid & 7) * tiles_per_xcd + (bid >> 3);
    if (tile >= tiles_total) return;
    const int tm = tile / tiles_n;
    const int tn = tile - tm * tiles_n;
    const int tid = threadIdx.x, lane = tid & 63, wave = tid >> 6;
    const int wm = wave / WGN, wn = wave % WGN;
    const int m0 = tm * BM, n0 = tn * BN;

    const i32x4_t rah = make_rsrc_words(p.Ah, a_bytes);
    const i32x4_t ral = make_rsrc_words(p.Al, a_bytes);
    const i32x4_t rw = make_rsrc_words(p.W, w_bytes);

    uint32_t a_voff[ACH], b_voff[BCH];
    int a_t[ACH];
    int a_len[ACH];
#pragma unroll
    for (int j = 0; j < ACH; ++j) {
        const int row = 16 * (wave * ACH + j) + (lane >> 2);
        const int seg = (lane & 3) ^ ((row >> 2) & 3);
        a_voff[j] = (m0 + row) < p.M ? (uint32_t)(((int64_t)(m0 + row) * p.lda + seg * 8) * 2) : OOB;
        a_t[j] = 0;
        a_len[j] = 0;
        if (CONV) {
            if (p.row_pos) {
                const int2 rp = (m0 + row) < p.M ? p.row_pos[m0 + row] : make_int2(0, 0);
                a_t[j] = rp.x;
                a_len[j] = rp.y;
            } else {
                a_t[j] = (m0 + row) % p.rows_per_item;
                a_len[j] = p.rows_per_item;
            }
        }
    }
    int nx_tap = 0, nx_cs = 0, nx_slab = 0;
    const int spt = CONV ? p.conv_cin / PBK : 1;
    const uint32_t row_bytes = (uint32_t)(p.lda * 2);
    uint32_t va_[ACH];
    int ka_ = 0;
#define PS_NEXT_ADDR()                                                                                  \
    do {                                                                                                \
        if (CONV) {                                                                                     \
            const int dt_ = nx_tap * p.conv_dil - p.conv_pad;                                           \
            ka_ = nx_cs * (PBK * 2);                                                                    \
            _Pragma("unroll") for (int j = 0; j < ACH; ++j) {                                           \
                const bool in_ = (uint32_t)(a_t[j] + dt_) < (uint32_t)a_len[j] && a_voff[j] != OOB;     \
                va_[j] = in_ ? a_voff[j] + (uint32_t)dt_ * row_bytes : OOB;                             \
            }                                                                                           \
// ... 301 lines not shown
                            if (v > am_best) {
                                am_best = v;
                                am_idx = col;
                            }
                        }
                    }
                }
            }
            return;
        }
        if (p.act == ACT_NONE) ps_epilogue<WM, EPN, EP_LD, ACT_NONE>(p, ep, m0w, n0w, lane);
        else if (p.act == ACT_RELU) ps_epilogue<WM, EPN, EP_LD, ACT_RELU>(p, ep, m0w, n0w, lane);
        else if (p.act == ACT_SILU) ps_epilogue<WM, EPN, EP_LD, ACT_SILU>(p, ep, m0w, n0w, lane);
        else ps_epilogue<WM, EPN, EP_LD, ACT_TANH>(p, ep, m0w, n0w, lane);
    };
    static_assert(WN % EPN == 0 && WN / EPN >= 1 && WN / EPN <= 4, "one to four epilogue passes");
    pass(std::integral_constant<int, 0>{});
    if constexpr (WN / EPN > 1) pass(std::integral_constant<int, 1>{});
    if constexpr (WN / EPN > 2) pass(std::integral_constant<int, 2>{});
    if constexpr (WN / EPN > 3) pass(std::integral_constant<int, 3>{});
    if constexpr (AMAX) {
        const int64_t m = m0w + lane;
        if (lane < WM && m < p.M) p.amax[m * p.amax_ld + tn * WGN + wn] = make_float2(am_best, __int_as_float(am_idx));
    }
}

template <int BM, int BN, int WGM, int WGN>
void launch_ps_cfg(const GemmPsArgs& a, hipStream_t s) {
    const int tiles_m = cdiv(a.M, BM), tiles_n = cdiv(a.N, BN);
    const int tiles_total = tiles_m * tiles_n;
    const int tiles_per_xcd = cdiv(tiles_total, 8);
    char name[64];
    snprintf(name, sizeof(name), "gemm_%dx%d_presplit", BM, BN);
    prof::Scope scope(name, 2.0 * a.M * (double)a.N * a.K,
                      4.0 * a.M * (double)a.K + 2.0 * a.N * (double)a.K + (a.amax ? 8.0 * a.M * (double)a.amax_ld : 4.0 * a.M * (double)a.N * (a.res ? 2.0 : 1.0)), s);
    const dim3 grid(tiles_per_xcd * 8), block(WGM * WGN * 64);
    const uint32_t ab = (uint32_t)((int64_t)a.M * a.lda * 2), wb = (uint32_t)((int64_t)a.N * a.ldw * 2);
    const auto launch = [&](auto kernel) { hipLaunchKernelGGL(kernel, grid, block, 0, s, a, tiles_n, tiles_total, tiles_per_xcd, ab, wb); };
    const bool conv = a.conv_taps > 0;
    if (a.amax) launch(gemm_ps_kernel<BM, BN, WGM, WGN, true, false, true>);
    else if (a.split && conv) launch(gemm_ps_kernel<BM, BN, WGM, WGN, true, true, false>);
    else if (a.split) launch(gemm_ps_kernel<BM, BN, WGM, WGN, true, false, false>);
    else if (conv) launch(gemm_ps_kernel<BM, BN, WGM, WGN, false, true, false>);
    else launch(gemm_ps_kernel<BM, BN, WGM, WGN, false, false, false>);
}

int ps_tile(int M, int N) {
    static const int max_tile = knob::value("SC_PS_TILE", 256);
    const int64_t tiles128 = (int64_t)cdiv(M, 128) * cdiv(N, 128);
    const int64_t tiles256 = (int64_t)cdiv(M, 256) * cdiv(N, 256);
    static const int min256 = knob::value("SC_PS_MIN256", 224);
    static const int min128 = knob::value("SC_PS_MIN128", 256);
    if (max_tile >= 256 && tiles256 >= min256 && N > 128) return 256;
    return tiles128 >= min128 ? 128 : 64;
}

}

void launch_gemm_presplit(const GemmPsArgs& a, hipStream_t s) {
    SC_CHECK(a.Ah && (a.Al || !a.split) && a.W && (a.C || a.Ch || a.amax), "presplit gemm: null operand");
    SC_CHECK(a.Ch || !a.Cl, "presplit gemm: a lo output plane needs its hi plane");
    SC_CHECK(a.M > 0 && a.N > 0 && a.K > 0 && a.K % PBK == 0, "presplit gemm: M=%d N=%d K=%d (K must be a multiple of 32)", a.M, a.N, a.K);
    SC_CHECK(a.lda % 8 == 0 && a.ldw % 8 == 0 && a.ldw >= a.K, "presplit gemm: lda=%lld ldw=%lld", (long long)a.lda,
             (long long)a.ldw);
    SC_CHECK(((reinterpret_cast<uintptr_t>(a.Ah) | reinterpret_cast<uintptr_t>(a.Al) | reinterpret_cast<uintptr_t>(a.W) |
               reinterpret_cast<uintptr_t>(a.C) | reinterpret_cast<uintptr_t>(a.res)) & 15) == 0 &&
                 ((reinterpret_cast<uintptr_t>(a.Ch) | reinterpret_cast<uintptr_t>(a.Cl)) & 7) == 0,
             "presplit gemm: operands must be 16-byte aligned");
    SC_CHECK((int64_t)a.M * a.lda * 2 < (1ll << 31) && (int64_t)a.N * a.ldw * 2 < (1ll << 31), "presplit gemm: operand larger than 2 GB");
    if (a.conv_taps > 0) {
        SC_CHECK(a.conv_cin % PBK == 0 && a.K == a.conv_taps * a.conv_cin && a.lda >= a.conv_cin &&
                     (a.row_pos || (a.rows_per_item > 0 && a.M % a.rows_per_item == 0)) && a.conv_dil >= 1 && a.conv_pad >= 0,
                 "presplit conv: taps=%d cin=%d K=%d rows_per_item=%d M=%d", a.conv_taps, a.conv_cin, a.K, a.rows_per_item, a.M);
    } else {
        SC_CHECK(a.lda >= a.K, "presplit gemm: lda=%lld < K=%d", (long long)a.lda, a.K);
    }
    if (a.amax) {
        SC_CHECK(a.split && a.conv_taps == 0 && !a.C && !a.Ch && !a.res && !a.row_valid && a.act == ACT_NONE,
                 "presplit gemm: the fused arg-max takes a plain product (no C / planes / residual / activation)");
        SC_CHECK(a.amax_ld == gemm_presplit_amax_chunks(a.M, a.N), "presplit gemm: amax_ld=%d, this shape produces %d partial results per row",
                 a.amax_ld, gemm_presplit_amax_chunks(a.M, a.N));
    }
    const int tile = ps_tile(a.M, a.N);
    if (tile == 256) launch_ps_cfg<256, 256, 4, 2>(a, s);
    else if (tile == 128) launch_ps_cfg<128, 128, 2, 2>(a, s);
    else launch_ps_cfg<64, 64, 2, 2>(a, s);
    SC_LAUNCH_CHECK();
}

int gemm_presplit_amax_chunks(int M, int N) { return 2 * cdiv(N, ps_tile(M, N)); }

namespace {
__global__ __launch_bounds__(256) void amax_finish_kernel(const float2* __restrict__ part, int ld, int rows, int* __restrict__ out_idx) {
    const int lane = threadIdx.x & 63;
    const int row = blockIdx.x * 4 + (threadIdx.x >> 6);
    if (row >= rows) return;
    const float2* pr = part + (int64_t)row * ld;
    float best = -INFINITY;
    int bidx = 0x7fffffff;
    for (int i = lane; i < ld; i += 64) {
        const float2 v = pr[i];
        const int vi = __float_as_int(v.y);
        if (v.x > best || (v.x == best && vi < bidx)) {
            best = v.x;
            bidx = vi;
        }
    }
#pragma unroll
    for (int o = 32; o > 0; o >>= 1) {
        const float ob = __shfl_xor(best, o);
        const int oi = __shfl_xor(bidx, o);
        if (ob > best || (ob == best && oi < bidx)) {
            best = ob;
            bidx = oi;
        }
    }
    if (lane == 0) out_idx[row] = bidx;
}
}

void launch_amax_finish(const float2* part, int ld, int rows, int* out_idx, hipStream_t s) {
    if (rows <= 0) return;
    hipLaunchKernelGGL(amax_finish_kernel, dim3(cdiv(rows, 4)), dim3(256), 0, s, part, ld, rows, out_idx);
    SC_LAUNCH_CHECK();
}

}
```

seamless_communication_amd/csrc/kernels.h:

```cpp
#pragma once
#include <atomic>

#include "common.h"
#include "prof.h"

namespace sc {

enum Act { ACT_NONE = 0, ACT_RELU = 1, ACT_SILU = 2, ACT_TANH = 3 };
enum InAct { IN_NONE = 0, IN_LRELU_01 = 1, IN_LRELU_001 = 2 };

struct GemmArgs {
    const float* A = nullptr;
    int64_t lda = 0;
    const __half* W = nullptr;
    int64_t ldw = 0;
    int64_t w_phase_stride = 0;
    const float* bias = nullptr;
    const float* res = nullptr;
    int64_t ldr = 0;
    float* C = nullptr;
    int64_t ldc = 0;
    int M = 0;
    int N = 0;
    int K = 0;
    int rows_per_batch = 0;
    int t_in = 0;
    int t_out = 0;
    int taps = 1, cin = 0, dil = 0, stride = 1, pad = 0;
    int out_mul = 1, out_off = 0, out_off_phase_step = 0;
    const int* in_lens = nullptr;
    int in_act = IN_NONE;
    int act = ACT_NONE;
    float alpha = 1.0f;
    int phases = 1;
    int split = 1;
    double algo_flops = 0;
    const int* item_off = nullptr;
    int n_items = 0, item_mul = 1, item_extra = 0, item_out_mul = 1;
};

#if defined(__HIPCC__)
template <typename F>
__device__ __forceinline__ int item_search(int n, int key, F first) {
    int lo = 0, hi = n - 1;
    while (lo < hi) {
        const int mid = (lo + hi + 1) >> 1;
        if (first(mid) <= key) lo = mid;
        else hi = mid - 1;
    }
    return lo;
}

struct GemmItemCursor {
    int n = 0, start = 0, next = 0x7fffffff;
    __device__ __forceinline__ static int first(const GemmArgs& p, int i) { return p.item_off[i] * p.item_mul + i * p.item_extra; }
    __device__ __forceinline__ void init(const GemmArgs& p, int m) {
        n = item_search(p.n_items, m, [&](int i) { return first(p, i); });
        start = first(p, n);
        next = first(p, n + 1);
    }
    __device__ __forceinline__ void seek(const GemmArgs& p, int m) {
        while (m >= next) {
            ++n;
            start = next;
            next = first(p, n + 1);
        }
    }
    __device__ __forceinline__ int q(int m) const { return m - start; }
    __device__ __forceinline__ int in_row0(const GemmArgs& p) const { return start - n * p.item_extra; }
    __device__ __forceinline__ int t_in(const GemmArgs& p) const { return next - start - p.item_extra; }
    __device__ __forceinline__ int t_out(const GemmArgs& p) const { return t_in(p) * p.item_out_mul; }
    __device__ __forceinline__ int64_t out_row0(const GemmArgs& p) const { return (int64_t)in_row0(p) * p.item_out_mul; }
};
#endif

void launch_gemm(const GemmArgs& a, hipStream_t s);
extern std::atomic<int> g_force_general_gemm;
bool gemm_fast_eligible(const GemmArgs& a);
void launch_gemm_fast(const GemmArgs& a, hipStream_t s);

struct GemmPsArgs {
    const __half* Ah = nullptr;
    const __half* Al = nullptr;
    int64_t lda = 0;
    const __half* W = nullptr;
    int64_t ldw = 0;
    const float* bias = nullptr;
    const float* res = nullptr;
    int64_t ldr = 0;
    float* C = nullptr;
    int64_t ldc = 0;
    __half* Ch = nullptr;
    __half* Cl = nullptr;
    int64_t ldcs = 0;
    int M = 0, N = 0, K = 0;
    int act = ACT_NONE;
    float alpha = 1.0f;
    int split = 1;
    float plane_neg_slope = 1.0f;
    int conv_taps = 0, conv_cin = 0, conv_dil = 1, conv_pad = 0, rows_per_item = 0;
    const unsigned char* row_valid = nullptr;
    const int2* row_pos = nullptr;
    float2* amax = nullptr;
    int amax_ld = 0;
};
void launch_gemm_presplit(const GemmPsArgs& a, hipStream_t s);
int gemm_presplit_amax_chunks(int M, int N);
void launch_amax_finish(const float2* part, int ld, int rows, int* out_idx, hipStream_t s);

struct ResPairArgs {
    const float* x = nullptr;
    float* out = nullptr;
    const __half* w1 = nullptr;
    int64_t ldw1 = 0;
    const float* b1 = nullptr;
    const __half* w2 = nullptr;
    int64_t ldw2 = 0;
    const float* b2 = nullptr;
    int nb = 0, T = 0, C = 0, k = 0, dil = 1;
    float slope = 0.1f;
    const float* avg_a = nullptr;
    const float* avg_b = nullptr;
    int single = 0;
    const int* item_off = nullptr;
    const int* tile_first = nullptr;
    int item_mul = 1, total_tiles = 0;
};
bool resblock_pair_supported(int C, int k, int dil);
int resblock_pair_tile_rows(int k);
void launch_resblock_pair(const ResPairArgs& a, hipStream_t s);

struct MrfArgs {
    const float* x = nullptr;
    float* out = nullptr;
    int nb = 0, T = 0, C = 0;
    float slope = 0.1f;
    int halo = 0;
    int k[3] = {0, 0, 0};
    int dil[9] = {1, 1, 1, 1, 1, 1, 1, 1, 1};
    const __half* w1[9] = {};
    const __half* w2[9] = {};
    int64_t ldw1[9] = {};
    int64_t ldw2[9] = {};
    const float* b1[9] = {};
    const float* b2[9] = {};
    int single = 0;
    const int* item_off = nullptr;
    const int* tile_first = nullptr;
    int item_mul = 1, total_tiles = 0;
};
bool mrf_fused_supported(int C, const int* k, const int* dil);
int mrf_tile_rows(const int* k, const int* dil);
void launch_mrf_fused(const MrfArgs& a, hipStream_t s);

void launch_gemv(const float* x, int64_t ldx, const __half* W, int64_t ldw, const float* bias,
                 const float* res, int64_t ldr, float* out, int64_t ldo, int M, int N, int K,
                 int act, float alpha, hipStream_t s);

struct SkinnyArgs {
    const float* A = nullptr;
    int64_t lda = 0;
    const __half* W = nullptr;
    int64_t ldw = 0;
    const float* bias = nullptr;
    const float* res = nullptr;
    int64_t ldr = 0;
    float* C = nullptr;
    int64_t ldc = 0;
    float* partial = nullptr;
    int M = 0, N = 0, K = 0;
    int act = ACT_NONE;
    float alpha = 1.0f;
    int splits = 1;
    int kc = 0;
    float4* am_part = nullptr;
    int am_tiles_cap = 0;
    int am_tiles = 0;
    float* am_eos_logit = nullptr;
    const int* am_pos = nullptr;
    int am_min_step_for_eos = 0, am_force_eos_step = -1;
    int am_pad_idx = -1, am_eos_idx = -1, am_unk_idx = -1;
    float am_unk_penalty = 0.f;
};
int skinny_argmax_tiles(int M, int N);
void launch_argmax_finalize(const float4* part, int tiles, int nb, const float* eos_logit, const int* d_pos,
                            int force_eos_step, int pad_idx, int eos_idx, int* next_tok, int* hist, int hist_ld,
                            int* finished, int* out_len, float* score, hipStream_t s);
void launch_skinny(const SkinnyArgs& a, hipStream_t s);
int skinny_splits(int M, int N, int K, int want_split);
// ... 127 lines not shown
    float* hfix = nullptr;
    int rows = 0, C = 0;
    const int* d_rows = nullptr;
    const int2* slot_rp = nullptr;
};
void launch_reduce3(const Reduce3Args& a, hipStream_t s);
void launch_embed3(const int* tok, const __half* embed, float scale, const float* pos_table, const int* d_pos, float* xg, int XRB,
                   int rows, int C, hipStream_t s, const int2* slot_rp = nullptr, const int* d_rows = nullptr);
void launch_ln3(const float* xg, int XRB, const float* gamma, const float* beta, __half* Hh, __half* Hl, int RB, int rows, int C,
                hipStream_t s);
void launch_rows_to_kgm(const float* x, int64_t ldx, int rows, int C, int XRB, float* xg, hipStream_t s);
void launch_kgm_to_rows(const float* xg, int XRB, float* out, int64_t ldo, int rows, int C, hipStream_t s);
struct Vocab3Args {
    const __half* Wp = nullptr;
    const __half* Ah = nullptr;
    const __half* Al = nullptr;
    int RB = 32;
    int M = 0, N = 0, K = 0;
    const float* bias = nullptr;
    float* logits = nullptr;
    int64_t ldl = 0;
    float4* am_part = nullptr;
    int am_tiles_cap = 0;
    float* am_eos_logit = nullptr;
    const int* am_pos = nullptr;
    int am_min_step_for_eos = 0, am_force_eos_step = -1;
    int am_pad_idx = -1, am_eos_idx = -1, am_unk_idx = -1;
    float am_unk_penalty = 0.f;
    const int* d_rows = nullptr;
    const int2* slot_rp = nullptr;
    const int* limit_row = nullptr;
    int KS = 0, NT_total = 0, tpg = 0, halves = 1;
    uint32_t w_bytes = 0;
};
bool vocab3_supported(int M, int N, int K);
int vocab3_groups(int M);
void launch_vocab3(const Vocab3Args& a, hipStream_t s);

void launch_layernorm(const float* x, int64_t ldx, const float* gamma, const float* beta, float* y,
                      int64_t ldy, int rows, int C, int act, const int* lens, int t_per_batch,
                      hipStream_t s);

void launch_layernorm_split(const float* x, int64_t ldx, const float* gamma, const float* beta, __half* yh, __half* yl,
                            int64_t ldh, int rows, int C, int act, const int* lens, int t_per_batch, hipStream_t s);
void launch_layernorm2_split(const float* x, int64_t ldx, const float* ga, const float* ba, float* y, int64_t ldy, const float* gb2,
                             const float* bb2, __half* yh, __half* yl, int64_t ldh, int rows, int C, hipStream_t s);
void launch_layernorm_both(const float* x, int64_t ldx, const float* gamma, const float* beta, float* y, int64_t ldy, __half* yh,
                           __half* yl, int64_t ldh, int rows, int C, int act, const int* lens, int t_per_batch, hipStream_t s);
void launch_lrelu_split_f32(const float* x, float neg_slope, __half* hi, __half* lo, int64_t n, hipStream_t s);
void launch_split_f32(const float* x, __half* hi, __half* lo, int64_t n, hipStream_t s);

void launch_glu(const float* x, int64_t ldx, float* y, int64_t ldy, int rows, int C, hipStream_t s);

bool glu_dwconv_ln_supported(int C, int ksize);
void launch_glu_dwconv_ln(const float* x, int64_t ldx, const float* w, const float* gamma, const float* beta, int act, __half* yh,
                          __half* yl, int64_t ldh, int nb, int T, int C, int ksize, const int* lens, hipStream_t s);
void launch_glu_dwconv(const float* x, int64_t ldx, const float* w, float* y, int64_t ldy, int nb, int T,
                       int C, int ksize, const int* lens, hipStream_t s, int left = -1, const float* bn_scale = nullptr,
                       const float* bn_shift = nullptr);
void launch_bn_fold(const float* g, const float* b, const float* mean, const float* var, float eps, int C, float* scale, float* shift,
                    hipStream_t s);
void launch_relpos_table(int S, int M, float* out, hipStream_t s);

struct AttnArgs {
    const float* q = nullptr;
    const float* k = nullptr;
    const float* v = nullptr;
    float* out = nullptr;
    int64_t ldq = 0, ldk = 0, ldv = 0, ldo = 0;
    int nb = 0, heads = 0, Sq = 0, Skv = 0;
    const int* kv_lens = nullptr;
    int causal = 0;
    const float* rel_k = nullptr;
    int rel_left = 0, rel_right = 0;
    const float* rp_table = nullptr;
    int64_t rp_ld = 0;
    const float* q_bias_u = nullptr;
    const float* q_bias_v = nullptr;
    const int* row_off = nullptr;
    double pairs = 0;
    __half* out_hi = nullptr;
    __half* out_lo = nullptr;
    int64_t ldoh = 0;
};
void launch_attention(const AttnArgs& a, hipStream_t s);

void launch_decode_attention(const float* q, int64_t ldq, const float* k_new, const float* v_new,
                             int64_t ldkv, float* kcache, float* vcache, int64_t cache_ld, int64_t cache_bs,
                             int cap, float* out, int64_t ldo, int nb, int heads, const int* d_pos,
                             const int* kv_lens, int use_lens, hipStream_t s, int in_splits = 1,
                             int64_t in_split_stride = 0, const float* bias_q = nullptr,
                             const float* bias_k = nullptr, const float* bias_v = nullptr);

constexpr int BANNED_MAX_SEQS = 4096, BANNED_MAX_LEN = 64, BANNED_MAX_TOKENS = 65536;
struct BannedList {
    const int* tokens = nullptr;
    const int* offsets = nullptr;
    int n = 0;
    int max_len = 0;
};
void validate_banned_host(const int32_t* tokens, const int32_t* offsets, int n_banned, int V, int* out_max_len);
void launch_beam_candidates(float* logits, int64_t ld, int n_utt, int beams, int V, const float* cum, int first_step,
                            int no_eos, int force_eos, int pad_idx, int eos_idx, int unk_idx, float unk_penalty, int K,
                            float* cand_val, int* cand_idx, const int* seqs, int seq_ld, int S, int G, hipStream_t s,
                            const int* d_slots = nullptr, const BannedList* banned = nullptr);
bool beam_chunked(int V, int beams, int K);
size_t beam_ws_floats(int rows, int K);
size_t beam_ws_ints(int rows, int K);
void launch_beam_candidates_chunked(float* logits, int64_t ld, int n_utt, int beams, int V, const float* cum, int first_step, int no_eos,
                                    int force_eos, int pad_idx, int eos_idx, int unk_idx, float unk_penalty, int K, float* cand_val,
                                    int* cand_idx, const int* seqs, int seq_ld, int S, int G, float* ws_f, int* ws_i, hipStream_t s,
                                    const int* d_rows = nullptr, const int* d_slots = nullptr, const BannedList* banned = nullptr);
struct BeamSelectArgs {
    const float* cand_val = nullptr;
    const int* cand_idx = nullptr;
    const int* seqs_cur = nullptr;
    int* seqs_new = nullptr;
    float* fin_score = nullptr;
    int* fin_len = nullptr;
    int* fin_seq = nullptr;
    int* fin_count = nullptr;
    int* done = nullptr;
    int* remaining = nullptr;
    int* tok = nullptr;
    int* src_row = nullptr;
    float* cum = nullptr;
    int* anc = nullptr;
    int anc_ld = 0;
    const int* slot_utt = nullptr;
    const int* d_slots = nullptr;
    int beams = 0, K = 0, V = 0, max_len = 0, step = 0;
    int eos_idx = 0, pad_idx = 0, normalize = 1;
    float len_penalty = 1.f;
};
void launch_beam_select(const BeamSelectArgs& a, int n_utt, hipStream_t s);
struct BeamCompactArgs {
    const int* done = nullptr;
    int* slot_utt = nullptr;
    int* d_slots = nullptr;
    int* d_rows = nullptr;
    int* seqs = nullptr;
    float* cum = nullptr;
    int* tok = nullptr;
    int* enc_lens = nullptr;
    int* anc = nullptr;
    int n = 0, beams = 0, max_len = 0, anc_ld = 0;
    int seq_len = 0, anc_len = 0;
};
void launch_beam_compact(const BeamCompactArgs& a, hipStream_t s);
void launch_row_token_lprob(const float* logits, int64_t ld, int rows, int V, int row_stride, int token, float* out, hipStream_t s);
void launch_gather_cache(const float* src, float* dst, const int* src_row, int rows, int len, int cap, int M, int layers,
                         int64_t layer_stride, hipStream_t s);

void launch_fbank(const float* wav, int64_t wav_stride, const int* num_samples, int nb, float* out,
                  int t_rows , const float* consts, float scale, hipStream_t s);
void launch_fbank_any(const float* wav, int64_t wav_stride, const int* num_samples, int nb, float* out, int t_rows, const float* consts,
                      float scale, int frame_len, int frame_shift, int nfft, hipStream_t s);
void launch_standardize(float* feat, int nb, int t_rows, const int* num_frames, int C, hipStream_t s);

void launch_embed_tokens(const int* tokens, int rows, const __half* emb, int M, float scale,
                         const float* pos_table, const int* d_pos, int t_per_batch, float* out,
                         int64_t ldo, hipStream_t s);
void launch_step_update(int* next_tok, int* hist, int hist_ld, int* finished, int* out_len,
                        const float* lprob, float* score, int nb, const int* d_pos, int pad_idx,
                        int eos_idx, int* n_unfinished, hipStream_t s);
void launch_argmax_rows(const float* logits, int64_t ld, int rows, int V, const int* d_pos,
// ... 123 lines not shown
```

seamless_communication_amd/csrc/model_encoder.hip:

```cpp
#include <cstdlib>

#include <cmath>
#include "model.h"

namespace sc {

static void upload_i32(Model& m, int* d, const int32_t* h, int n) {
    SC_HIP(hipMemcpyAsync(d, h, (size_t)n * 4, hipMemcpyHostToDevice, m.stream));
}

static void fbank_geometry(int sample_rate, int& frame_len, int& frame_shift, int& nfft) {
    frame_len = (int)((float)sample_rate * 0.001f * 25.0f);
    frame_shift = (int)((float)sample_rate * 0.001f * 10.0f);
    nfft = 1;
    while (nfft < frame_len) nfft *= 2;
}

int fbank_num_frames(int64_t num_samples, int sample_rate) {
    int fl, fs, nf;
    fbank_geometry(sample_rate, fl, fs, nf);
    return num_samples < fl ? 0 : (int)(1 + (num_samples - fl) / fs);
}

static const Model::FbankRate& fbank_rate_consts(Model& m, int sample_rate) {
// ... 56 lines not shown
    if (standardize) launch_standardize(d_out, n, t_rows, d_fr, m.cfg.num_fbank_channels, m.stream);
    SC_HIP(hipStreamSynchronize(m.stream));
}

static int adaptor_len(const sc_config& c, int len) {
    const int pad = c.adaptor_kernel_size / 2;
    const double v = (double)(len + 2 * pad - c.adaptor_kernel_size) / (double)c.adaptor_stride + 1.0;
    return (int)std::floor(v);
}

int encoder_out_len(const Model& m, int t_frames) {
    const sc_config& c = m.cfg;
    const int S = t_frames / c.fbank_stride;
    const int pad = c.adaptor_kernel_size / 2;
    return (S + 2 * pad - c.adaptor_kernel_size) / c.adaptor_stride + 1;
}

static void attention_self(Model& m, const float* qkv, int Mdim, float* out, int nb, int S, const int* d_lens,
                           const float* rel_k) {
    AttnArgs a;
    a.q = qkv;
    a.k = qkv + Mdim;
    a.v = qkv + 2 * Mdim;
    a.out = out;
    a.ldq = a.ldk = a.ldv = 3 * Mdim;
    a.ldo = Mdim;
    a.nb = nb;
    a.heads = m.cfg.num_heads;
    a.Sq = S;
    a.Skv = S;
    a.kv_lens = d_lens;
    a.rel_k = rel_k;
    a.rel_left = rel_k ? m.cfg.shaw_max_left : 0;
    a.rel_right = rel_k ? m.cfg.shaw_max_right : 0;
    launch_attention(a, m.stream);
}

void run_encode_speech(Model& m, const float* d_fbank, int n, int t_frames, const int32_t* h_lens, float* d_out,
                       int32_t* h_out_lens) {
    const sc_config& c = m.cfg;
    const int M = c.model_dim;
    SC_CHECK(n > 0 && t_frames > 0, "sc_encode_speech: empty batch");
    prof::set_tag("enc");
    SC_CHECK(t_frames % c.fbank_stride == 0, "sc_encode_speech: t_frames=%d must be a multiple of fbank_stride=%d (Collater pad_to_multiple)",
             t_frames, c.fbank_stride);
    const int S = t_frames / c.fbank_stride;
    const int rows = n * S;
    const int feat = c.num_fbank_channels * c.fbank_stride;
    std::vector<int32_t> lens(n), alens(n);
    for (int i = 0; i < n; ++i) {
        SC_CHECK(h_lens[i] >= 0 && h_lens[i] <= t_frames, "sc_encode_speech: frame_lens[%d]=%d out of range", i, h_lens[i]);
        lens[i] = h_lens[i] / c.fbank_stride;
        alens[i] = adaptor_len(c, lens[i]);
        if (h_out_lens) h_out_lens[i] = alens[i];
    }
    Buf<int> d_lens(m.pp(), n), d_alens(m.pp(), n);
    upload_i32(m, d_lens, lens.data(), n);
    upload_i32(m, d_alens, alens.data(), n);

    const int F = std::max(std::max(c.enc_ffn_dim, c.adaptor_proj_dim), std::max(3 * M, c.adaptor_ffn_dim));
    Buf<float> x(m.pp(), (size_t)rows * M), h(m.pp(), (size_t)rows * std::max(M, feat)), wide(m.pp(), (size_t)rows * F),
        att(m.pp(), (size_t)rows * M);

    launch_layernorm(d_fbank, feat, m.fe_ln.g, m.fe_ln.b, h, feat, rows, feat, ACT_NONE, nullptr, 1, m.stream);
    linear(m, h, feat, m.fe_proj, nullptr, 0, x, M, rows, ACT_NONE, 1.f);

    static const bool presplit = knob::value("SC_PRESPLIT", 1) != 0;
    const bool v1 = c.enc_variant == 1;
    const bool ps_ok = !v1 && presplit && M % 32 == 0 && c.enc_ffn_dim % 32 == 0 && (int64_t)rows * std::max(M, c.enc_ffn_dim) * 2 < (1ll << 31);
    Buf<float> rp_tab(m.pp(), v1 ? (size_t)(2 * S - 1) * M : 0), rp_proj(m.pp(), v1 ? (size_t)(2 * S - 1) * M : 0);
    if (v1) launch_relpos_table(S, M, rp_tab, m.stream);
    Buf<__half> hs(m.pp(), ps_ok ? (size_t)2 * rows * M : 0), ws(m.pp(), ps_ok ? (size_t)2 * rows * c.enc_ffn_dim : 0),
        as(m.pp(), ps_ok ? (size_t)2 * rows * M : 0);
    __half* hs_hi = hs.get();
    __half* hs_lo = ps_ok ? hs.get() + (size_t)rows * M : nullptr;
    __half* ws_hi = ws.get();
    __half* ws_lo = ps_ok ? ws.get() + (size_t)rows * c.enc_ffn_dim : nullptr;
    __half* as_hi = as.get();
    __half* as_lo = ps_ok ? as.get() + (size_t)rows * M : nullptr;
    auto ln_split = [&](const float* src, const LNorm& L, int act) {
        launch_layernorm_split(src, L.dim, L.g, L.b, hs_hi, hs_lo, L.dim, rows, L.dim, act, nullptr, 1, m.stream);
    };
    auto ps = [&](const __half* ah, const __half* al, const Linear& L, int act, float alpha, const float* res, float* C,
                  __half* Ch, __half* Cl) {
        GemmPsArgs a;
        a.Ah = ah;
        a.Al = al;
        a.lda = L.in;
        a.W = L.w;
        a.ldw = L.ldw;
        a.bias = L.b;
        a.res = res;
        a.ldr = L.out;
        a.C = C;
        a.ldc = L.out;
        a.Ch = Ch;
        a.Cl = Cl;
        a.ldcs = L.out;
        a.M = rows;
        a.N = L.out;
        a.K = L.in;
        a.act = act;
        a.alpha = alpha;
        static const bool single = knob::value("SC_SPLIT_MODE", 0) == 1;
        a.split = single ? 0 : 1;
        launch_gemm_presplit(a, m.stream);
    };

    static const bool fuse = knob::value("SC_ENC_FUSE", 1) != 0;
    const bool fuse_conv = fuse && glu_dwconv_ln_supported(M, c.depthwise_conv_kernel_size);
    const bool fuse_ln = fuse && M <= 1024;
    bool ffn1_planes_ready = false;
    for (int li = 0; li < c.enc_layers; ++li) {
        const ConformerLayer& l = m.enc[li];
        if (ps_ok) {
            if (!ffn1_planes_ready) ln_split(x, l.ffn1_ln, ACT_NONE);
            ps(hs_hi, hs_lo, l.ffn1_in, ACT_SILU, 1.f, nullptr, nullptr, ws_hi, ws_lo);
            ps(ws_hi, ws_lo, l.ffn1_out, ACT_NONE, 0.5f, x, x, nullptr, nullptr);
            ln_split(x, l.attn_ln, ACT_NONE);
            ps(hs_hi, hs_lo, l.qkv, ACT_NONE, 1.f, nullptr, wide, nullptr, nullptr);
            {
                AttnArgs a;
                a.q = wide;
                a.k = wide.get() + M;
                a.v = wide.get() + 2 * M;
                a.out_hi = as_hi;
                a.out_lo = as_lo;
                a.ldoh = M;
                a.ldq = a.ldk = a.ldv = 3 * M;
                a.ldo = M;
                a.nb = n;
                a.heads = c.num_heads;
                a.Sq = S;
                a.Skv = S;
                a.kv_lens = d_lens;
                a.rel_k = l.rel_k;
                a.rel_left = c.shaw_max_left;
                a.rel_right = c.shaw_max_right;
                launch_attention(a, m.stream);
            }
            ps(as_hi, as_lo, l.attn_out, ACT_NONE, 1.f, x, x, nullptr, nullptr);
            ln_split(x, l.conv_ln, ACT_NONE);
            ps(hs_hi, hs_lo, l.pw1, ACT_NONE, 1.f, nullptr, wide, nullptr, nullptr);
            if (fuse_conv) {
                launch_glu_dwconv_ln(wide, 2 * M, l.dw, l.conv_inner_ln.g, l.conv_inner_ln.b, ACT_SILU, hs_hi, hs_lo, M, n, S, M,
                                     c.depthwise_conv_kernel_size, d_lens, m.stream);
            } else {
                launch_glu_dwconv(wide, 2 * M, l.dw, att, M, n, S, M, c.depthwise_conv_kernel_size, d_lens, m.stream);
                ln_split(att, l.conv_inner_ln, ACT_SILU);
            }
            ps(hs_hi, hs_lo, l.pw2, ACT_NONE, 1.f, x, x, nullptr, nullptr);
            ln_split(x, l.ffn2_ln, ACT_NONE);
            ps(hs_hi, hs_lo, l.ffn2_in, ACT_SILU, 1.f, nullptr, nullptr, ws_hi, ws_lo);
            ps(ws_hi, ws_lo, l.ffn2_out, ACT_NONE, 0.5f, x, x, nullptr, nullptr);
            if (fuse_ln && li + 1 < c.enc_layers) {
                const LNorm& nx = m.enc[li + 1].ffn1_ln;
                launch_layernorm2_split(x, M, l.final_ln.g, l.final_ln.b, x, M, nx.g, nx.b, hs_hi, hs_lo, M, rows, M, m.stream);
                ffn1_planes_ready = true;
            } else {
                layernorm(m, x, l.final_ln, x, rows);
                ffn1_planes_ready = false;
            }
            continue;
        }
        layernorm(m, x, l.ffn1_ln, h, rows);
        linear(m, h, M, l.ffn1_in, nullptr, 0, wide, c.enc_ffn_dim, rows, ACT_SILU, 1.f);
        linear(m, wide, c.enc_ffn_dim, l.ffn1_out, x, M, x, M, rows, ACT_NONE, 0.5f);
        layernorm(m, x, l.attn_ln, h, rows);
        linear(m, h, M, l.qkv, nullptr, 0, wide, 3 * M, rows, ACT_NONE, 1.f);
        if (v1) {
            linear(m, rp_tab, M, l.r_proj, nullptr, 0, rp_proj, M, 2 * S - 1, ACT_NONE, 1.f);
            AttnArgs a;
            a.q = wide;
            a.k = wide.get() + M;
            a.v = wide.get() + 2 * M;
            a.out = att;
            a.ldq = a.ldk = a.ldv = 3 * M;
            a.ldo = M;
            a.nb = n;
            a.heads = c.num_heads;
            a.Sq = S;
            a.Skv = S;
            a.kv_lens = d_lens;
            a.rp_table = rp_proj;
            a.rp_ld = M;
            a.q_bias_u = l.u_bias;
            a.q_bias_v = l.v_bias;
            launch_attention(a, m.stream);
        } else {
            attention_self(m, wide, M, att, n, S, d_lens, l.rel_k);
        }
        linear(m, att, M, l.attn_out, x, M, x, M, rows, ACT_NONE, 1.f);
        layernorm(m, x, l.conv_ln, h, rows);
        linear(m, h, M, l.pw1, nullptr, 0, wide, 2 * M, rows, ACT_NONE, 1.f);
        if (v1) {
            launch_glu_dwconv(wide, 2 * M, l.dw, h, M, n, S, M, c.depthwise_conv_kernel_size, d_lens, m.stream,
                              c.depthwise_conv_kernel_size / 2, l.bn_scale, l.bn_shift);
        } else {
            launch_glu_dwconv(wide, 2 * M, l.dw, att, M, n, S, M, c.depthwise_conv_kernel_size, d_lens, m.stream);
            layernorm(m, att, l.conv_inner_ln, h, rows, ACT_SILU);
        }
        linear(m, h, M, l.pw2, x, M, x, M, rows, ACT_NONE, 1.f);
        layernorm(m, x, l.ffn2_ln, h, rows);
        linear(m, h, M, l.ffn2_in, nullptr, 0, wide, c.enc_ffn_dim, rows, ACT_SILU, 1.f);
        linear(m, wide, c.enc_ffn_dim, l.ffn2_out, x, M, x, M, rows, ACT_NONE, 0.5f);
        layernorm(m, x, l.final_ln, x, rows);
    }
    layernorm(m, x, m.enc_inner_ln, x, rows);
// ... 27 lines not shown
```

seamless_communication_amd/csrc/model_t2u.hip:

```cpp
#include <cstdlib>

#include "model.h"

namespace sc {

namespace {

void attention_self(Model& m, const float* qkv, int M, float* out, int nb, int S, const int* d_lens) {
    AttnArgs a;
    a.q = qkv;
    a.k = qkv + M;
    a.v = qkv + 2 * M;
    a.out = out;
    a.ldq = a.ldk = a.ldv = 3 * M;
    a.ldo = M;
    a.nb = nb;
    a.heads = m.cfg.num_heads;
    a.Sq = S;
    a.Skv = S;
    a.kv_lens = d_lens;
    launch_attention(a, m.stream);
}

void text_to_char_seqs(const Model& m, const int32_t* text_seqs, int n, int s_text, std::vector<int32_t>& char_lens,
// ... 213 lines not shown
        SC_HIP(hipStreamSynchronize(m.stream));
    }

    int Su = 0;
    std::vector<int32_t> ulens(n);
    for (int b = 0; b < n; ++b) {
        int64_t tot = 0;
        for (int k = 0; k < Sc; ++k) tot += dur[(size_t)b * Sc + k];
        SC_CHECK(tot <= c.unit_max_seq_len, "sc_t2u_nar: %lld units exceed unit_max_seq_len=%d", (long long)tot, c.unit_max_seq_len);
        ulens[b] = (int)tot;
        Su = std::max(Su, ulens[b]);
        if (h_unit_lens) h_unit_lens[b] = ulens[b];
    }
    SC_CHECK(Su > 0, "sc_t2u_nar: zero units predicted");
    const int urows = n * Su;
    Buf<int> d_ulens(m.pp(), n);
    SC_HIP(hipMemcpyAsync(d_ulens.get(), ulens.data(), (size_t)n * 4, hipMemcpyHostToDevice, m.stream));

    std::vector<int32_t> ids((size_t)urows, c.unit_pad_idx);
    static const int max_groups = std::max(1, knob::value("SC_T2U_GROUPS", 8));
    const std::vector<std::vector<int>> groups = plan_length_groups(std::vector<int>(ulens.begin(), ulens.end()), 400, max_groups);
    int64_t rows_done = 0;
    auto finish = [&](const std::vector<int32_t>& unit_ids, int64_t rows_computed) {
        m.last_padded_unit_rows = rows_computed;
        m.last_units.assign((size_t)urows, 0);
        for (int b = 0; b < n; ++b)
            for (int t = 0; t < Su; ++t) {
                int32_t v = t < ulens[b] ? unit_ids[(size_t)b * Su + t] : c.unit_pad_idx;
                if (v == c.unit_eos_idx) v = c.unit_pad_idx;
                if (v == c.unit_pad_idx) v = c.unit_pad_idx + 4;
                m.last_units[(size_t)b * Su + t] = v - 4;
            }
        m.last_durations = dur;
        m.last_char_ids = cid_flat;
        m.last_char_seq_lens = cseq_lens;
        m.last_n = n;
        m.last_su = Su;
        m.last_sc = Sc;
        if (out_su) *out_su = Su;
        if (out_sc) *out_sc = Sc;
    };
    {
        static const bool want_packed = knob::value("SC_T2U_PACKED", 1) != 0;
        const int K = c.t2u_conv_kernel, Ci = c.t2u_conv_inner_dim;
        int64_t R64 = 0;
        for (int b = 0; b < n; ++b) R64 += ulens[b];
        const bool packed = want_packed && M % 32 == 0 && Ci % 32 == 0 && K % 2 == 1 && !m.t2u_dec.empty() && M == c.num_heads * 64 &&
                            m.t2u_dec[0].conv1.kpad == M * K && m.t2u_dec[0].conv2.kpad == Ci * K &&
                            R64 * std::max(M, Ci) * 2 < (1ll << 31) && R64 * (int64_t)c.unit_vocab_size < (1ll << 31);
        if (packed) {
            const int R = (int)R64;
            std::vector<int32_t> uidx((size_t)R), row_t((size_t)R), row_off(n), pos2((size_t)2 * R);
            int r = 0;
            for (int b = 0; b < n; ++b) {
                row_off[b] = r;
                int t = 0;
                for (int k = 0; k < Sc; ++k)
                    for (int q = 0; q < dur[(size_t)b * Sc + k]; ++q, ++t, ++r) {
                        uidx[r] = b * Sc + k;
                        row_t[r] = t;
                        pos2[(size_t)2 * r] = t;
                        pos2[(size_t)2 * r + 1] = ulens[b];
                    }
            }
            Buf<int> d_uidx(m.pp(), R), d_row_t(m.pp(), R), d_row_off(m.pp(), n), d_pos2(m.pp(), (size_t)2 * R), d_ids(m.pp(), R);
            SC_HIP(hipMemcpyAsync(d_uidx.get(), uidx.data(), (size_t)R * 4, hipMemcpyHostToDevice, m.stream));
            SC_HIP(hipMemcpyAsync(d_row_t.get(), row_t.data(), (size_t)R * 4, hipMemcpyHostToDevice, m.stream));
            SC_HIP(hipMemcpyAsync(d_row_off.get(), row_off.data(), (size_t)n * 4, hipMemcpyHostToDevice, m.stream));
            SC_HIP(hipMemcpyAsync(d_pos2.get(), pos2.data(), (size_t)2 * R * 4, hipMemcpyHostToDevice, m.stream));
            const int2* d_row_pos = reinterpret_cast<const int2*>(d_pos2.get());
            double pairs = 0;
            for (int b = 0; b < n; ++b) pairs += (double)ulens[b] * ulens[b];
            const int wideN = 3 * M;
            Buf<float> u(m.pp(), (size_t)R * M), y(m.pp(), (size_t)R * M), wide(m.pp(), (size_t)R * wideN);
            Buf<__half> planes(m.pp(), (size_t)R * (6 * M + 2 * Ci));
            __half* up_h = planes.get();
            __half* up_l = up_h + (size_t)R * M;
            __half* yp_h = up_l + (size_t)R * M;
            __half* yp_l = yp_h + (size_t)R * M;
            __half* ap_h = yp_l + (size_t)R * M;
            __half* ap_l = ap_h + (size_t)R * M;
            __half* wp_h = ap_l + (size_t)R * M;
            __half* wp_l = wp_h + (size_t)R * Ci;
            auto ps = [&](const __half* ah, const __half* al, const Linear& L, const float* res, float* C) {
                GemmPsArgs a;
                a.Ah = ah;
                a.Al = al;
                a.lda = L.in;
                a.W = L.w;
                a.ldw = L.ldw;
                a.bias = L.b;
                a.res = res;
                a.ldr = L.out;
                a.C = C;
                a.ldc = L.out;
                a.M = R;
                a.N = L.out;
                a.K = L.in;
                launch_gemm_presplit(a, m.stream);
            };
            launch_gather_rows(cs, M, d_uidx, u, M, R, M, m.stream);
            launch_pos_add_rows(u, M, m.unit_pos, d_row_t, m.pos_alpha, R, M, m.stream);
            launch_split_f32(u, up_h, up_l, (int64_t)R * M, m.stream);
            for (const FFTLayer& l : m.t2u_dec) {
                ps(up_h, up_l, l.qkv, nullptr, wide);
                AttnArgs a;
                a.q = wide;
                a.k = wide.get() + M;
                a.v = wide.get() + 2 * M;
                a.out_hi = ap_h;
                a.out_lo = ap_l;
                a.ldoh = M;
                a.ldq = a.ldk = a.ldv = 3 * M;
                a.ldo = M;
                a.nb = n;
                a.heads = c.num_heads;
                a.Sq = Su;
                a.Skv = Su;
                a.kv_lens = d_ulens;
                a.row_off = d_row_off;
                a.pairs = pairs;
                launch_attention(a, m.stream);
                ps(ap_h, ap_l, l.attn_out, u, y);
                launch_layernorm_both(y, M, l.attn_ln.g, l.attn_ln.b, y, M, yp_h, yp_l, M, R, M, ACT_NONE, nullptr, 1, m.stream);
                conv1d_presplit(m, yp_h, yp_l, l.conv1, nullptr, nullptr, wp_h, wp_l, 0, 0, K / 2, 1, nullptr, ACT_RELU, R, d_row_pos);
                conv1d_presplit(m, wp_h, wp_l, l.conv2, y, u, nullptr, nullptr, 0, 0, K / 2, 1, nullptr, ACT_NONE, R, d_row_pos);
                launch_layernorm_both(u, M, l.conv_ln.g, l.conv_ln.b, u, M, up_h, up_l, M, R, M, ACT_NONE, nullptr, 1, m.stream);
            }
            launch_layernorm_split(u, M, m.t2u_dec_ln.g, m.t2u_dec_ln.b, up_h, up_l, M, R, M, ACT_NONE, nullptr, 1, m.stream);
            const int nch = gemm_presplit_amax_chunks(R, c.unit_vocab_size);
            Buf<float2> part(m.pp(), (size_t)R * nch);
            GemmPsArgs a;
            a.Ah = up_h;
            a.Al = up_l;
            a.lda = M;
            a.W = m.unit_embed;
            a.ldw = M;
            a.M = R;
            a.N = c.unit_vocab_size;
            a.K = M;
            a.amax = part;
            a.amax_ld = nch;
            launch_gemm_presplit(a, m.stream);
            launch_amax_finish(part, nch, R, d_ids, m.stream);
            std::vector<int32_t> pids((size_t)R);
            SC_HIP(hipMemcpyAsync(pids.data(), d_ids.get(), (size_t)R * 4, hipMemcpyDeviceToHost, m.stream));
            SC_HIP(hipStreamSynchronize(m.stream));
            std::vector<int32_t> ids((size_t)urows, c.unit_pad_idx);
            for (int b = 0; b < n; ++b)
                for (int t = 0; t < ulens[b]; ++t) ids[(size_t)b * Su + t] = pids[(size_t)row_off[b] + t];
            finish(ids, R);
            return;
        }
    }
    std::vector<std::vector<int32_t>> keep_alive;
    std::vector<Buf<int>> id_bufs;
    keep_alive.reserve(3 * groups.size());
    for (const std::vector<int>& grp : groups) {
        const int ng = (int)grp.size();
        int Lg = 0;
        for (int b : grp) Lg = std::max(Lg, ulens[b]);
        const int grows = ng * Lg;
        rows_done += grows;
        keep_alive.emplace_back((size_t)grows, -1);
        std::vector<int32_t>& uidx = keep_alive.back();
        keep_alive.emplace_back((size_t)ng);
        std::vector<int32_t>& glens = keep_alive.back();
        for (int gi = 0; gi < ng; ++gi) {
            const int b = grp[gi];
            glens[gi] = ulens[b];
            int pos = 0;
            for (int k = 0; k < Sc; ++k)
                for (int r = 0; r < dur[(size_t)b * Sc + k]; ++r) uidx[(size_t)gi * Lg + pos++] = b * Sc + k;
        }
        Buf<int> d_uidx(m.pp(), grows), d_glens(m.pp(), ng);
        id_bufs.emplace_back(m.pp(), grows);
        int* d_ids = id_bufs.back();
        SC_HIP(hipMemcpyAsync(d_uidx.get(), uidx.data(), (size_t)grows * 4, hipMemcpyHostToDevice, m.stream));
        SC_HIP(hipMemcpyAsync(d_glens.get(), glens.data(), (size_t)ng * 4, hipMemcpyHostToDevice, m.stream));
        Buf<float> u(m.pp(), (size_t)grows * M), y(m.pp(), (size_t)grows * M), att(m.pp(), (size_t)grows * M),
            wide(m.pp(), (size_t)grows * wideN);
        launch_gather_rows(cs, M, d_uidx, u, M, grows, M, m.stream);
        launch_pos_add(u, M, m.unit_pos, Lg, m.pos_alpha, grows, M, m.stream);
        const int K = c.t2u_conv_kernel;
        for (const FFTLayer& l : m.t2u_dec) {
            linear(m, u, M, l.qkv, nullptr, 0, wide, 3 * M, grows, ACT_NONE, 1.f);
            attention_self(m, wide, M, att, ng, Lg, d_glens);
            linear(m, att, M, l.attn_out, u, M, y, M, grows, ACT_NONE, 1.f);
            layernorm(m, y, l.attn_ln, y, grows);
            conv1d(m, y, l.conv1, nullptr, wide, ng, Lg, 1, K / 2, 1, d_glens, IN_NONE, ACT_RELU);
            conv1d(m, wide, l.conv2, y, u, ng, Lg, 1, K / 2, 1, d_glens, IN_NONE, ACT_NONE);
            layernorm(m, u, l.conv_ln, u, grows);
// ... 495 lines not shown
```

Before: 338.1.

## Feed self-attention K/V as fp16 hi/lo planes emitted by the QKV GEMM

The presplit QKV GEMM epilogue now also writes the K and V column range as fp16 hi/lo planes, starting at a tile-aligned plane_col0. A new attention kernel variant loads these planes directly into double-buffered LDS tiles and reads V with transposing LDS reads. This removes the per-tile fp32-to-fp16 split of K/V inside attention and overlaps global loads with compute. The cost is extra plane writes from the GEMM, reuse of scratch buffers (ws / yp / wp) that must not be live at the time, and more LDS per workgroup. It is enabled by default in the Conformer encoder and the NAR T2U decoder.

```diff
diff --git a/include/seamless_hip.h b/include/seamless_hip.h
--- a/include/seamless_hip.h
+++ b/include/seamless_hip.h
@@ -8,7 +8,7 @@
 extern "C" {
 #endif
 
-#define SC_ABI_VERSION 10
+#define SC_ABI_VERSION 11
 #define SC_MAX_UPSAMPLES 8
 #define SC_MAX_RESBLOCK_KERNELS 4
 #define SC_MAX_RESBLOCK_DILATIONS 4
diff --git a/include/seamless_hip_internal.h b/include/seamless_hip_internal.h
--- a/include/seamless_hip_internal.h
+++ b/include/seamless_hip_internal.h
@@ -76,6 +76,14 @@
                        const int32_t* d_kv_lens, int32_t causal, const float* d_rel_k, int32_t rel_left,
                        int32_t rel_right, const int32_t* d_row_off, const float* d_rp_table, int64_t rp_ld,
                        const float* d_q_bias_u, const float* d_q_bias_v, void* d_out_hi, void* d_out_lo, int64_t ldoh);
+int sc_op_attention_kv_planes(const float* d_q, const void* d_k_hi, const void* d_k_lo, const void* d_v_hi, const void* d_v_lo,
+                              int64_t ldkh, float* d_out, int32_t nb, int32_t heads, int32_t sq, int32_t skv, int64_t ldq, int64_t ldo,
+                              const int32_t* d_kv_lens, int32_t causal, const float* d_rel_k, int32_t rel_left, int32_t rel_right,
+                              const int32_t* d_row_off, void* d_out_hi, void* d_out_lo, int64_t ldoh);
+int sc_op_split_f32(const float* d_x, void* d_hi_f16, void* d_lo_f16, int64_t n);
+int sc_op_linear_presplit_bound(const float* d_x, const void* d_w_f16, const float* d_bias, const float* d_res, float* d_y,
+                                void* d_yh_f16, void* d_yl_f16, int32_t M, int32_t N, int32_t K, int32_t act, float alpha,
+                                int32_t plane_col0);
 int sc_op_glu_dwconv(const float* d_x, const float* d_w, float* d_y, int32_t nb, int32_t T, int32_t C, int32_t k,
                      const int32_t* d_lens);
 int sc_op_glu_dwconv_ln(const float* d_x, const float* d_w, const float* d_gamma, const float* d_beta, int32_t act, void* d_yh_f16,
diff --git a/seamless_communication_amd/_lib.py b/seamless_communication_amd/_lib.py
--- a/seamless_communication_amd/_lib.py
+++ b/seamless_communication_amd/_lib.py
@@ -9,7 +9,7 @@
 _VARIANT = os.environ.get("SC_LIB_VARIANT", "")
 LIB_PATH = Path(__file__).resolve().parent / (f"libseamless_hip.{_VARIANT}.so" if _VARIANT else "libseamless_hip.so")
 
-SC_ABI_VERSION = 10
+SC_ABI_VERSION = 11
 SC_MAX_UPSAMPLES = 8
 SC_MAX_RESBLOCK_KERNELS = 4
 SC_MAX_RESBLOCK_DILATIONS = 4
@@ -184,6 +184,10 @@
                                   _P, _i, _i]),
     "sc_op_attention_ex": (C.c_int, [_P, _P, _P, _P, _i, _i, _i, _i, C.c_int64, C.c_int64, C.c_int64, C.c_int64, _P, _i,
                                      _P, _i, _i, _P, _P, C.c_int64, _P, _P, _P, _P, C.c_int64]),
+    "sc_op_attention_kv_planes": (C.c_int, [_P, _P, _P, _P, _P, C.c_int64, _P, _i, _i, _i, _i, C.c_int64, C.c_int64, _P, _i, _P, _i, _i,
+                                            _P, _P, _P, C.c_int64]),
+    "sc_op_split_f32": (C.c_int, [_P, _P, _P, C.c_int64]),
+    "sc_op_linear_presplit_bound": (C.c_int, [_P, _P, _P, _P, _P, _P, _P, _i, _i, _i, _i, C.c_float, _i]),
     "sc_op_glu_dwconv": (C.c_int, [_P, _P, _P, _i, _i, _i, _i, _P]),
     "sc_op_argmax": (C.c_int, [_P, _i, _i, _P, _P]),
     "sc_op_beam_candidates": (C.c_int, [_P, C.c_int64, _i, _i, _i, _P, _i, _i, _i, _i, _i, _i, C.c_float, _i, _P, _P, _P, _i, _i, _i,
diff --git a/seamless_communication_amd/csrc/api.hip b/seamless_communication_amd/csrc/api.hip
--- a/seamless_communication_amd/csrc/api.hip
+++ b/seamless_communication_amd/csrc/api.hip
@@ -1136,6 +1136,20 @@
 
 int sc_op_linear_presplit(const float* d_x, const void* d_w_f16, const float* d_bias, const float* d_res, float* d_y,
                           void* d_yh_f16, void* d_yl_f16, int32_t M, int32_t N, int32_t K, int32_t act, float alpha) {
+    return sc_op_linear_presplit_bound(d_x, d_w_f16, d_bias, d_res, d_y, d_yh_f16, d_yl_f16, M, N, K, act, alpha, 0);
+}
+
+int sc_op_split_f32(const float* d_x, void* d_hi_f16, void* d_lo_f16, int64_t n) {
+    SC_API_BEGIN
+    SC_CHECK(d_x && d_hi_f16 && d_lo_f16 && n > 0 && n % 4 == 0, "sc_op_split_f32: null argument or n not a multiple of 4");
+    launch_split_f32(d_x, static_cast<__half*>(d_hi_f16), static_cast<__half*>(d_lo_f16), n, g_op_stream);
+    SC_HIP(hipStreamSynchronize(g_op_stream));
+    SC_API_END
+}
+
+int sc_op_linear_presplit_bound(const float* d_x, const void* d_w_f16, const float* d_bias, const float* d_res, float* d_y,
+                                void* d_yh_f16, void* d_yl_f16, int32_t M, int32_t N, int32_t K, int32_t act, float alpha,
+                                int32_t plane_col0) {
     SC_API_BEGIN
     SC_CHECK(d_x && d_w_f16 && (d_y || d_yh_f16), "sc_op_linear_presplit: null argument");
     __half *hi = nullptr, *lo = nullptr;
@@ -1156,7 +1170,8 @@
         a.ldc = N;
         a.Ch = static_cast<__half*>(d_yh_f16);
         a.Cl = static_cast<__half*>(d_yl_f16);
-        a.ldcs = N;
+        a.ldcs = N - plane_col0;
+        a.plane_col0 = plane_col0;
         a.M = M;
         a.N = N;
         a.K = K;
@@ -1378,6 +1393,40 @@
     a.rp_ld = rp_ld;
     a.q_bias_u = d_q_bias_u;
     a.q_bias_v = d_q_bias_v;
+    a.out_hi = static_cast<__half*>(d_out_hi);
+    a.out_lo = static_cast<__half*>(d_out_lo);
+    a.ldoh = ldoh;
+    launch_attention(a, g_op_stream);
+    SC_HIP(hipStreamSynchronize(g_op_stream));
+    SC_API_END
+}
+
+int sc_op_attention_kv_planes(const float* d_q, const void* d_k_hi, const void* d_k_lo, const void* d_v_hi, const void* d_v_lo,
+                              int64_t ldkh, float* d_out, int32_t nb, int32_t heads, int32_t sq, int32_t skv, int64_t ldq, int64_t ldo,
+                              const int32_t* d_kv_lens, int32_t causal, const float* d_rel_k, int32_t rel_left, int32_t rel_right,
+                              const int32_t* d_row_off, void* d_out_hi, void* d_out_lo, int64_t ldoh) {
+    SC_API_BEGIN
+    SC_CHECK(d_q && d_k_hi && d_k_lo && d_v_hi && d_v_lo, "sc_op_attention_kv_planes: null argument");
+    AttnArgs a;
+    a.q = d_q;
+    a.k_hi = static_cast<const __half*>(d_k_hi);
+    a.k_lo = static_cast<const __half*>(d_k_lo);
+    a.v_hi = static_cast<const __half*>(d_v_hi);
+    a.v_lo = static_cast<const __half*>(d_v_lo);
+    a.ldkh = ldkh;
+    a.out = d_out;
+    a.ldq = ldq;
+    a.ldo = ldo;
+    a.nb = nb;
+    a.heads = heads;
+    a.Sq = sq;
+    a.Skv = skv;
+    a.kv_lens = d_kv_lens;
+    a.causal = causal;
+    a.rel_k = d_rel_k;
+    a.rel_left = rel_left;
+    a.rel_right = rel_right;
+    a.row_off = d_row_off;
     a.out_hi = static_cast<__half*>(d_out_hi);
     a.out_lo = static_cast<__half*>(d_out_lo);
     a.ldoh = ldoh;
diff --git a/seamless_communication_amd/csrc/common.cpp b/seamless_communication_amd/csrc/common.cpp
--- a/seamless_communication_amd/csrc/common.cpp
+++ b/seamless_communication_amd/csrc/common.cpp
@@ -35,6 +35,7 @@
     {"SC_PS_TILE", 0, "DMA GEMM: largest tile"}, {"SC_PS_MIN256", 0, "DMA GEMM: tiles needed for 256 x 256"},
     {"SC_PS_MIN128", 0, "DMA GEMM: tiles needed for 128 x 128"},
     {"SC_PRESPLIT", 0, "0: Conformer operands split on the fly"}, {"SC_ENC_FUSE", 0, "0: separate Conformer element-wise launches"},
+    {"SC_ATTN_KV_PLANES", 0, "0: self-attention of the encoder / NAR decoder reads K / V as fp32 rows instead of the QKV product's fp16 planes"},
     {"SC_D3_RG_SMALL", 0, "decoder step: rows per row group, N = 1024 products"}, {"SC_D3_RG_FFN", 0, "decoder step: rows per row group, FFN-in"},
     {"SC_G3_STATIONARY", 0, "row-group products of wide steps: 0 one workgroup per row group, n = workgroup budget of the weight-stationary launch"},
     {"SC_G3_TILES", 0, "0: FFN-out of wide steps on the weight-stationary row-group walk instead of tile-owning waves"},
diff --git a/seamless_communication_amd/csrc/k_attn.hip b/seamless_communication_amd/csrc/k_attn.hip
--- a/seamless_communication_amd/csrc/k_attn.hip
+++ b/seamless_communication_amd/csrc/k_attn.hip
@@ -13,6 +13,18 @@
 typedef _Float16 a16_h4 __attribute__((ext_vector_type(4)));
 static constexpr int KH_LD = 72;
 static constexpr int VT_LD = 40;
+static constexpr int KVP_TILE = 2 * MKV * KH_LD + 2 * MKV * HD;
+static_assert(2 * KVP_TILE * 2 <= 4 * 32 * KS * 4, "the two tile buffers fit the region the output tiles use afterwards");
+typedef unsigned int a16_u4 __attribute__((ext_vector_type(4)));
+
+__device__ __forceinline__ a16_h4 a16_read_tr(const _Float16* lds_ptr) {
+    typedef short s4_t __attribute__((__vector_size__(8)));
+    typedef __attribute__((address_space(3))) s4_t lds_s4_t;
+    const s4_t v = __builtin_amdgcn_ds_read_tr16_b64_v4i16((lds_s4_t*)(lds_ptr));
+    a16_h4 r;
+    __builtin_memcpy(&r, &v, 8);
+    return r;
+}
 
 __device__ __forceinline__ void a16_split8(const float* x, a16_h8& hi, a16_h8& lo) {
 #pragma unroll
@@ -23,10 +35,11 @@
     }
 }
 
-template <int MODE>
-__global__ __launch_bounds__(256) void attn_mfma16_kernel(AttnArgs p) {
+template <int MODE, bool KVP>
+__device__ __forceinline__ void attn_mfma16_body(const AttnArgs& p) {
     constexpr bool SHAW = MODE == 1;
     constexpr bool RELPOS = MODE == 2;
+    static_assert(!(KVP && RELPOS), "the planes mode serves MODE 0 and 1");
     typedef float f16v __attribute__((ext_vector_type(16)));
     typedef float f4v __attribute__((ext_vector_type(4)));
     extern __shared__ __attribute__((aligned(16))) float smem[];
@@ -157,9 +170,43 @@
             }
         }
     };
-    if (k_end > 0) fetch(0);
+    const int pr = tid >> 3, pc = tid & 7;
+    a16_u4 g[4];
+    auto fetch_planes = [&](int k0) {
+#pragma unroll
+        for (int u = 0; u < 4; ++u) g[u] = a16_u4{0u, 0u, 0u, 0u};
+        if (k0 + pr < kv_len) {
+            const int64_t off = (kvbase + k0 + pr) * p.ldkh + h * HD + pc * 8;
+            g[0] = *reinterpret_cast<const a16_u4*>(p.k_hi + off);
+            g[1] = *reinterpret_cast<const a16_u4*>(p.k_lo + off);
+            g[2] = *reinterpret_cast<const a16_u4*>(p.v_hi + off);
+            g[3] = *reinterpret_cast<const a16_u4*>(p.v_lo + off);
+        }
+    };
+    auto store_planes = [&](int buf) {
+        _Float16* t = sKh + buf * KVP_TILE;
+        *reinterpret_cast<a16_u4*>(t + pr * KH_LD + pc * 8) = g[0];
+        *reinterpret_cast<a16_u4*>(t + MKV * KH_LD + pr * KH_LD + pc * 8) = g[1];
+        const int vo = pr * HD + ((pc * 8) ^ (((pr >> 1) & 1) << 5));
+        *reinterpret_cast<a16_u4*>(t + 2 * MKV * KH_LD + vo) = g[2];
+        *reinterpret_cast<a16_u4*>(t + 2 * MKV * KH_LD + MKV * HD + vo) = g[3];
+    };
+    const int vq = (lane & 15) >> 2;
+    const int vt_off = (4 * hh + vq) * HD + ((((vq >> 1) & 1) << 5) | (((lane >> 4) & 1) << 4) | ((lane & 3) << 2));
+    if constexpr (KVP) {
+        if (k_end > 0) fetch_planes(0);
+        __syncthreads();
+        if (k_end > 0) store_planes(0);
+    } else {
+        if (k_end > 0) fetch(0);
+    }
 
     for (int k0 = 0; k0 < k_end; k0 += MKV) {
+        const int buf = KVP ? ((k0 / MKV) & 1) : 0;
+        if constexpr (KVP) {
+            if (k0 + MKV < k_end) fetch_planes(k0 + MKV);
+            __syncthreads();
+        } else {
         __syncthreads();
 #pragma unroll
         for (int u = 0; u < 2; ++u) {
@@ -186,6 +233,9 @@
         }
         if (k0 + MKV < k_end) fetch(k0 + MKV);
         __syncthreads();
+        }
+        const _Float16* tKh = sKh + buf * KVP_TILE;
+        const _Float16* tKl = KVP ? tKh + MKV * KH_LD : sKl;
 
         float qr[16];
         if (SHAW) {
@@ -254,8 +304,8 @@
         for (int r = 0; r < 16; ++r) st[r] = 0.f;
 #pragma unroll
         for (int c = 0; c < 4; ++c) {
-            const a16_h8 kh = *reinterpret_cast<const a16_h8*>(&sKh[ql * KH_LD + 16 * c + 8 * hh]);
-            const a16_h8 kl = *reinterpret_cast<const a16_h8*>(&sKl[ql * KH_LD + 16 * c + 8 * hh]);
+            const a16_h8 kh = *reinterpret_cast<const a16_h8*>(&tKh[ql * KH_LD + 16 * c + 8 * hh]);
+            const a16_h8 kl = *reinterpret_cast<const a16_h8*>(&tKl[ql * KH_LD + 16 * c + 8 * hh]);
             st = __builtin_amdgcn_mfma_f32_32x32x16_f16(kh, qh[c], st, 0, 0, 0);
             st = __builtin_amdgcn_mfma_f32_32x32x16_f16(kh, qlo[c], st, 0, 0, 0);
             st = __builtin_amdgcn_mfma_f32_32x32x16_f16(kl, qh[c], st, 0, 0, 0);
@@ -299,10 +349,22 @@
             for (int e = 0; e < 8; ++e) x[e] = st[8 * c + e];
             a16_h8 ph, pl;
             a16_split8(x, ph, pl);
-            const a16_h8 v0h = *reinterpret_cast<const a16_h8*>(&sVh[ql * VT_LD + 16 * c + 8 * hh]);
-            const a16_h8 v0l = *reinterpret_cast<const a16_h8*>(&sVl[ql * VT_LD + 16 * c + 8 * hh]);
-            const a16_h8 v1h = *reinterpret_cast<const a16_h8*>(&sVh[(32 + ql) * VT_LD + 16 * c + 8 * hh]);
-            const a16_h8 v1l = *reinterpret_cast<const a16_h8*>(&sVl[(32 + ql) * VT_LD + 16 * c + 8 * hh]);
+            a16_h8 v0h, v0l, v1h, v1l;
+            if constexpr (KVP) {
+                const _Float16* tv = tKh + 2 * MKV * KH_LD + 16 * c * HD;
+                const auto rd = [&](const _Float16* pl, int x) {
+                    return __builtin_shufflevector(a16_read_tr(pl + (vt_off ^ x)), a16_read_tr(pl + 8 * HD + (vt_off ^ x)), 0, 1, 2, 3, 4, 5, 6, 7);
+                };
+                v0h = rd(tv, 0);
+                v0l = rd(tv + MKV * HD, 0);
+                v1h = rd(tv, 32);
+                v1l = rd(tv + MKV * HD, 32);
+            } else {
+                v0h = *reinterpret_cast<const a16_h8*>(&sVh[ql * VT_LD + 16 * c + 8 * hh]);
+                v0l = *reinterpret_cast<const a16_h8*>(&sVl[ql * VT_LD + 16 * c + 8 * hh]);
+                v1h = *reinterpret_cast<const a16_h8*>(&sVh[(32 + ql) * VT_LD + 16 * c + 8 * hh]);
+                v1l = *reinterpret_cast<const a16_h8*>(&sVl[(32 + ql) * VT_LD + 16 * c + 8 * hh]);
+            }
             o0 = __builtin_amdgcn_mfma_f32_32x32x16_f16(v0h, ph, o0, 0, 0, 0);
             o1 = __builtin_amdgcn_mfma_f32_32x32x16_f16(v1h, ph, o1, 0, 0, 0);
             o0 = __builtin_amdgcn_mfma_f32_32x32x16_f16(v0h, pl, o0, 0, 0, 0);
@@ -310,6 +372,8 @@
             o0 = __builtin_amdgcn_mfma_f32_32x32x16_f16(v0l, ph, o0, 0, 0, 0);
             o1 = __builtin_amdgcn_mfma_f32_32x32x16_f16(v1l, ph, o1, 0, 0, 0);
         }
+        if constexpr (KVP)
+            if (k0 + MKV < k_end) store_planes(buf ^ 1);
     }
 
     __syncthreads();
@@ -340,6 +404,16 @@
     }
 }
 
+template <int MODE>
+__global__ __launch_bounds__(256) void attn_mfma16_kernel(AttnArgs p) {
+    attn_mfma16_body<MODE, false>(p);
+}
+
+template <int MODE>
+__global__ __launch_bounds__(256) void attn_mfma16_planes_kernel(AttnArgs p) {
+    attn_mfma16_body<MODE, true>(p);
+}
+
 static bool g_attn_attr_set = false;
 
 void launch_attention(const AttnArgs& a, hipStream_t s) {
@@ -350,6 +424,13 @@
     const int npos = a.rel_left + 1 + a.rel_right;
     SC_CHECK(npos <= 96, "attention: %d relative positions > 96", npos);
     SC_CHECK(!a.row_off || (a.kv_lens && a.Sq == a.Skv && !a.causal), "attention: packed rows need kv_lens and Sq == Skv");
+    const bool kvp = a.k_hi != nullptr;
+    if (kvp) {
+        SC_CHECK(a.k_lo && a.v_hi && a.v_lo && !a.rp_table, "attention: the planes mode needs all four K / V planes and serves MODE 0 / 1");
+        SC_CHECK(a.ldkh % 8 == 0 && ((reinterpret_cast<uintptr_t>(a.k_hi) | reinterpret_cast<uintptr_t>(a.k_lo) | reinterpret_cast<uintptr_t>(a.v_hi) |
+                                      reinterpret_cast<uintptr_t>(a.v_lo)) & 15) == 0,
+                 "attention: K / V planes must be 16-byte aligned with a row stride that is a multiple of 8");
+    }
     if (a.rp_table)
         SC_CHECK(!a.rel_k && !a.causal && a.Sq == a.Skv && a.q_bias_u && a.q_bias_v && a.rp_ld % 4 == 0,
                  "attention: relative positions need self-attention (Sq == Skv), both query biases and a 16-byte aligned table");
@@ -357,6 +438,8 @@
         SC_HIP(hipFuncSetAttribute(reinterpret_cast<const void*>(&attn_mfma16_kernel<0>), hipFuncAttributeMaxDynamicSharedMemorySize, 120 * 1024));
         SC_HIP(hipFuncSetAttribute(reinterpret_cast<const void*>(&attn_mfma16_kernel<1>), hipFuncAttributeMaxDynamicSharedMemorySize, 120 * 1024));
         SC_HIP(hipFuncSetAttribute(reinterpret_cast<const void*>(&attn_mfma16_kernel<2>), hipFuncAttributeMaxDynamicSharedMemorySize, 120 * 1024));
+        SC_HIP(hipFuncSetAttribute(reinterpret_cast<const void*>(&attn_mfma16_planes_kernel<0>), hipFuncAttributeMaxDynamicSharedMemorySize, 120 * 1024));
+        SC_HIP(hipFuncSetAttribute(reinterpret_cast<const void*>(&attn_mfma16_planes_kernel<1>), hipFuncAttributeMaxDynamicSharedMemorySize, 120 * 1024));
         g_attn_attr_set = true;
     }
     const double pairs = a.pairs > 0 ? a.pairs : (double)a.nb * a.Sq * a.Skv;
@@ -366,7 +449,9 @@
     if (a.rel_k) lds += (size_t)(MQ * npos) * sizeof(float);
     if (a.rp_table) lds += (size_t)(4 * 64 * 32) * sizeof(float);
     dim3 grid(cdiv(a.Sq, MQ), a.heads, a.nb);
-    if (a.rp_table) hipLaunchKernelGGL((attn_mfma16_kernel<2>), grid, dim3(256), lds, s, a);
+    if (kvp && a.rel_k) hipLaunchKernelGGL((attn_mfma16_planes_kernel<1>), grid, dim3(256), lds, s, a);
+    else if (kvp) hipLaunchKernelGGL((attn_mfma16_planes_kernel<0>), grid, dim3(256), lds, s, a);
+    else if (a.rp_table) hipLaunchKernelGGL((attn_mfma16_kernel<2>), grid, dim3(256), lds, s, a);
     else if (a.rel_k) hipLaunchKernelGGL((attn_mfma16_kernel<1>), grid, dim3(256), lds, s, a);
     else hipLaunchKernelGGL((attn_mfma16_kernel<0>), grid, dim3(256), lds, s, a);
     SC_LAUNCH_CHECK();
diff --git a/seamless_communication_amd/csrc/k_gemm_ps.hip b/seamless_communication_amd/csrc/k_gemm_ps.hip
--- a/seamless_communication_amd/csrc/k_gemm_ps.hip
+++ b/seamless_communication_amd/csrc/k_gemm_ps.hip
@@ -50,6 +50,12 @@
     const int c0 = (rank % LPR) * 4;
     const int col = n0w + c0;
     const bool vec_ok = (col + 3 < p.N) && ((p.ldc | p.ldr | p.ldcs) % 4 == 0) && (n0w % 4 == 0);
+    const bool bound = p.plane_col0 > 0;
+    const bool right = bound && n0w >= p.plane_col0;
+    float* const C = right ? nullptr : p.C;
+    _Float16* const Ch = (bound && !right) ? nullptr : reinterpret_cast<_Float16*>(p.Ch);
+    _Float16* const Cl = (bound && !right) ? nullptr : reinterpret_cast<_Float16*>(p.Cl);
+    const int pcol = right ? col - p.plane_col0 : col;
     f4_t b4 = {0.f, 0.f, 0.f, 0.f};
     if (p.bias) {
 #pragma unroll
@@ -67,16 +73,16 @@
         for (int e = 0; e < 4; ++e) v[e] = dead ? 0.f : ps_act<ACT>(a[e] + b4[e]) * p.alpha;
         if (vec_ok) {
             if (p.res && !dead) v += *reinterpret_cast<const f4_t*>(p.res + m * p.ldr + col);
-            if (p.C) *reinterpret_cast<f4_t*>(p.C + m * p.ldc + col) = v;
-            if (p.Ch) {
+            if (C) *reinterpret_cast<f4_t*>(C + m * p.ldc + col) = v;
+            if (Ch) {
                 if (p.plane_neg_slope != 1.0f) {
 #pragma unroll
                     for (int e = 0; e < 4; ++e) v[e] = fmaxf(v[e], 0.f) + p.plane_neg_slope * fminf(v[e], 0.f);
                 }
                 const h4_t hi = __builtin_convertvector(v, h4_t);
-                *reinterpret_cast<h4_t*>(reinterpret_cast<_Float16*>(p.Ch) + m * p.ldcs + col) = hi;
-                if (p.Cl)
-                    *reinterpret_cast<h4_t*>(reinterpret_cast<_Float16*>(p.Cl) + m * p.ldcs + col) =
+                *reinterpret_cast<h4_t*>(Ch + m * p.ldcs + pcol) = hi;
+                if (Cl)
+                    *reinterpret_cast<h4_t*>(Cl + m * p.ldcs + pcol) =
                         __builtin_convertvector(v - __builtin_convertvector(hi, f4_t), h4_t);
             }
         } else {
@@ -85,12 +91,12 @@
                 if (col + e >= p.N) continue;
                 float x = v[e];
                 if (p.res && !dead) x += p.res[m * p.ldr + col + e];
-                if (p.C) p.C[m * p.ldc + col + e] = x;
-                if (p.Ch) {
+                if (C) C[m * p.ldc + col + e] = x;
+                if (Ch) {
                     if (p.plane_neg_slope != 1.0f) x = fmaxf(x, 0.f) + p.plane_neg_slope * fminf(x, 0.f);
                     const _Float16 h = (_Float16)x;
-                    reinterpret_cast<_Float16*>(p.Ch)[m * p.ldcs + col + e] = h;
-                    if (p.Cl) reinterpret_cast<_Float16*>(p.Cl)[m * p.ldcs + col + e] = (_Float16)(x - (float)h);
+                    Ch[m * p.ldcs + pcol + e] = h;
+                    if (Cl) Cl[m * p.ldcs + pcol + e] = (_Float16)(x - (float)h);
                 }
             }
         }
@@ -558,11 +564,16 @@
                  a.amax_ld, gemm_presplit_amax_chunks(a.M, a.N));
     }
     const int tile = ps_tile(a.M, a.N);
+    if (a.plane_col0 != 0)
+        SC_CHECK(a.plane_col0 > 0 && a.plane_col0 < a.N && a.plane_col0 % tile == 0 && a.C && a.Ch && !a.amax,
+                 "presplit gemm: plane_col0=%d must be a multiple of the %d-wide tile inside N=%d, with C and planes given", a.plane_col0, tile, a.N);
     if (tile == 256) launch_ps_cfg<256, 256, 4, 2>(a, s);
     else if (tile == 128) launch_ps_cfg<128, 128, 2, 2>(a, s);
     else launch_ps_cfg<64, 64, 2, 2>(a, s);
     SC_LAUNCH_CHECK();
 }
+
+int gemm_presplit_tile(int M, int N) { return ps_tile(M, N); }
 
 int gemm_presplit_amax_chunks(int M, int N) { return 2 * cdiv(N, ps_tile(M, N)); }
 
diff --git a/seamless_communication_amd/csrc/kernels.h b/seamless_communication_amd/csrc/kernels.h
--- a/seamless_communication_amd/csrc/kernels.h
+++ b/seamless_communication_amd/csrc/kernels.h
@@ -103,8 +103,10 @@
     const int2* row_pos = nullptr;
     float2* amax = nullptr;
     int amax_ld = 0;
+    int plane_col0 = 0;
 };
 void launch_gemm_presplit(const GemmPsArgs& a, hipStream_t s);
+int gemm_presplit_tile(int M, int N);
 int gemm_presplit_amax_chunks(int M, int N);
 void launch_amax_finish(const float2* part, int ld, int rows, int* out_idx, hipStream_t s);
 
@@ -398,6 +400,11 @@
     __half* out_hi = nullptr;
     __half* out_lo = nullptr;
     int64_t ldoh = 0;
+    const __half* k_hi = nullptr;
+    const __half* k_lo = nullptr;
+    const __half* v_hi = nullptr;
+    const __half* v_lo = nullptr;
+    int64_t ldkh = 0;
 };
 void launch_attention(const AttnArgs& a, hipStream_t s);
 
diff --git a/seamless_communication_amd/csrc/model_encoder.hip b/seamless_communication_amd/csrc/model_encoder.hip
--- a/seamless_communication_amd/csrc/model_encoder.hip
+++ b/seamless_communication_amd/csrc/model_encoder.hip
@@ -162,7 +162,7 @@
         launch_layernorm_split(src, L.dim, L.g, L.b, hs_hi, hs_lo, L.dim, rows, L.dim, act, nullptr, 1, m.stream);
     };
     auto ps = [&](const __half* ah, const __half* al, const Linear& L, int act, float alpha, const float* res, float* C,
-                  __half* Ch, __half* Cl) {
+                  __half* Ch, __half* Cl, int plane_col0 = 0) {
         GemmPsArgs a;
         a.Ah = ah;
         a.Al = al;
@@ -176,7 +176,8 @@
         a.ldc = L.out;
         a.Ch = Ch;
         a.Cl = Cl;
-        a.ldcs = L.out;
+        a.ldcs = L.out - plane_col0;
+        a.plane_col0 = plane_col0;
         a.M = rows;
         a.N = L.out;
         a.K = L.in;
@@ -190,6 +191,8 @@
     static const bool fuse = knob::value("SC_ENC_FUSE", 1) != 0;
     const bool fuse_conv = fuse && glu_dwconv_ln_supported(M, c.depthwise_conv_kernel_size);
     const bool fuse_ln = fuse && M <= 1024;
+    static const bool kv_planes_knob = knob::value("SC_ATTN_KV_PLANES", 1) != 0;
+    const bool kv_planes = ps_ok && kv_planes_knob && c.enc_ffn_dim >= 2 * M && M % gemm_presplit_tile(rows, 3 * M) == 0;
     bool ffn1_planes_ready = false;
     for (int li = 0; li < c.enc_layers; ++li) {
         const ConformerLayer& l = m.enc[li];
@@ -198,12 +201,18 @@
             ps(hs_hi, hs_lo, l.ffn1_in, ACT_SILU, 1.f, nullptr, nullptr, ws_hi, ws_lo);
             ps(ws_hi, ws_lo, l.ffn1_out, ACT_NONE, 0.5f, x, x, nullptr, nullptr);
             ln_split(x, l.attn_ln, ACT_NONE);
-            ps(hs_hi, hs_lo, l.qkv, ACT_NONE, 1.f, nullptr, wide, nullptr, nullptr);
+            if (kv_planes) ps(hs_hi, hs_lo, l.qkv, ACT_NONE, 1.f, nullptr, wide, ws_hi, ws_lo, M);
+            else ps(hs_hi, hs_lo, l.qkv, ACT_NONE, 1.f, nullptr, wide, nullptr, nullptr);
             {
                 AttnArgs a;
                 a.q = wide;
                 a.k = wide.get() + M;
                 a.v = wide.get() + 2 * M;
+                if (kv_planes) {
+                    a.k_hi = ws_hi, a.k_lo = ws_lo;
+                    a.v_hi = ws_hi + M, a.v_lo = ws_lo + M;
+                    a.ldkh = 2 * M;
+                }
                 a.out_hi = as_hi;
                 a.out_lo = as_lo;
                 a.ldoh = M;
diff --git a/seamless_communication_amd/csrc/model_t2u.hip b/seamless_communication_amd/csrc/model_t2u.hip
--- a/seamless_communication_amd/csrc/model_t2u.hip
+++ b/seamless_communication_amd/csrc/model_t2u.hip
@@ -319,7 +319,11 @@
             __half* ap_l = ap_h + (size_t)R * M;
             __half* wp_h = ap_l + (size_t)R * M;
             __half* wp_l = wp_h + (size_t)R * Ci;
-            auto ps = [&](const __half* ah, const __half* al, const Linear& L, const float* res, float* C) {
+            static const bool kv_planes_knob = knob::value("SC_ATTN_KV_PLANES", 1) != 0;
+            const bool kv_planes = kv_planes_knob && Ci >= M && M % gemm_presplit_tile(R, 3 * M) == 0;
+            __half* kv_h = yp_h;
+            __half* kv_l = wp_h;
+            auto ps = [&](const __half* ah, const __half* al, const Linear& L, const float* res, float* C, int plane_col0 = 0) {
                 GemmPsArgs a;
                 a.Ah = ah;
                 a.Al = al;
@@ -331,6 +335,7 @@
                 a.ldr = L.out;
                 a.C = C;
                 a.ldc = L.out;
+                if (plane_col0 > 0) a.Ch = kv_h, a.Cl = kv_l, a.ldcs = L.out - plane_col0, a.plane_col0 = plane_col0;
                 a.M = R;
                 a.N = L.out;
                 a.K = L.in;
@@ -340,11 +345,16 @@
             launch_pos_add_rows(u, M, m.unit_pos, d_row_t, m.pos_alpha, R, M, m.stream);
             launch_split_f32(u, up_h, up_l, (int64_t)R * M, m.stream);
             for (const FFTLayer& l : m.t2u_dec) {
-                ps(up_h, up_l, l.qkv, nullptr, wide);
+                ps(up_h, up_l, l.qkv, nullptr, wide, kv_planes ? M : 0);
                 AttnArgs a;
                 a.q = wide;
                 a.k = wide.get() + M;
                 a.v = wide.get() + 2 * M;
+                if (kv_planes) {
+                    a.k_hi = kv_h, a.k_lo = kv_l;
+                    a.v_hi = kv_h + M, a.v_lo = kv_l + M;
+                    a.ldkh = 2 * M;
+                }
                 a.out_hi = ap_h;
                 a.out_lo = ap_l;
                 a.ldoh = M;
```

After: 341.7, median of 6. +1.1%, better.
